# experimental-design/everest

Hardware: AMD Instinct MI355X
Metric: QnehviStrategy.ask() candidates/sec + GP posterior ms, n=512 d=6 m=5 (higher is better)
Workload: dtype f64; 1 GPU; full QnehviStrategy.ask() of BASELINE configs[3] (config 4): DTLZ2(d=6,m=5), n_train=512, S=256 MC samples, 1024 raw Sobol candidates + 20 L-BFGS-B restarts, q=1; value = (raw + optimiser evaluations x batch) / ask wall time, SURVEY.md §8(d); n_train=512, d=6, m=5, mc_samples=256, raw_samples=1024, restarts=20, batch_limit=20, parallelism=1 rank

## Files before the change

### everest_amd/_native.py

```python
from __future__ import annotations

import ctypes
import os
from ctypes import POINTER, c_char_p, c_double, c_int, c_longlong, c_void_p

import torch

_HERE = os.path.dirname(os.path.abspath(__file__))
LIB_PATH = os.environ.get("EVR_LIB_PATH") or os.path.join(_HERE, "_lib", "libeverest_amd.so")

c_double_p = c_void_p
c_int_p = c_void_p


class NativeLibraryError(RuntimeError):
    pass


class EvrQnehviState(ctypes.Structure):
    _fields_ = [
        ("n", c_int), ("nb", c_int), ("S", c_int), ("m", c_int),
        ("c", c_void_p), ("ym", c_void_p), ("ys", c_void_p), ("kxx", c_void_p),
        ("zq", c_void_p), ("obj_a", c_void_p), ("obj_b", c_void_p),
        ("cell_lo", c_void_p), ("cell_hi", c_void_p), ("cell_off", c_void_p), ("max_cells", c_int),
        ("cell_keys", c_void_p), ("cell_pts", c_void_p), ("cell_rank0", c_void_p), ("pts_stride", c_int),
        ("grp_off", c_void_p), ("grp_keys", c_void_p), ("grp_rank", c_void_p), ("grp_box", c_void_p),
        ("sorted_lo", c_void_p), ("max_groups", c_int), ("scan_counters", c_void_p), ("no_h", c_int),
        ("log_hvi", c_int), ("tau_relu", c_double), ("tau_max", c_double),
    ]


class EvrQnehviModel(ctypes.Structure):
    _fields_ = [
        ("n", c_int), ("d", c_int), ("kind", c_int),
        ("Xn", c_void_p), ("lengthscales", c_void_p), ("shift", c_void_p), ("scale", c_void_p), ("M", c_void_p),
    ]


class EvrQnGeneral(ctypes.Structure):
    _fields_ = [
        ("q", c_int), ("m_obj", c_int),
        ("obj_out", c_void_p), ("obj_kind", c_void_p), ("obj_p0", c_void_p), ("obj_p1", c_void_p),
        ("n_con", c_int),
        ("con_out", c_void_p), ("con_sign", c_void_p), ("con_thr", c_void_p), ("con_eta", c_void_p),
        ("zq", c_void_p),
    ]

class EvrNei(ctypes.Structure):
    _fields_ = [
        ("log", c_int), ("tau_relu", c_double), ("tau_max", c_double), ("best", c_void_p), ("best_stride", c_int),
    ]


class EvrSobo(ctypes.Structure):
    _fields_ = [
        ("log", c_int), ("tau_relu", c_double), ("tau_max", c_double), ("best", c_void_p), ("best_stride", c_int),
        ("n_term", c_int),
        ("term_out", c_void_p), ("term_kind", c_void_p), ("term_w", c_void_p), ("term_p0", c_void_p),
        ("term_p1", c_void_p), ("term_p2", c_void_p),
        ("n_con", c_int),
        ("con_out", c_void_p), ("con_sign", c_void_p), ("con_thr", c_void_p), ("con_eta", c_void_p),
    ]


_SIGS = {
    "evr_version": ([], c_int),
    "evr_last_error": ([], c_char_p),
    "evr_device_arch": ([c_int, c_char_p, c_int], c_int),
    "evr_stream_sync": ([c_void_p], c_int),
    "evr_kernel_matrix": ([c_void_p, c_int, c_int, c_int, c_int, c_int] + [c_void_p] * 10, c_int),
    "evr_kernel_cross_grad": ([c_void_p, c_int, c_int, c_int, c_int, c_int] + [c_void_p] * 11, c_int),
    "evr_kernel_cross_grad_workspace_doubles": ([c_int, c_int, c_int], c_longlong),
    "evr_kernel_lengthscale_grad": ([c_void_p, c_int, c_int, c_int, c_int, c_void_p, c_void_p, c_void_p,
                                     c_void_p, c_void_p], c_int),
    "evr_gp_mll_terms": ([c_void_p, c_int, c_int] + [c_void_p] * 5, c_int),
    "evr_gemm_f64": ([c_void_p, c_int, c_int, c_int, c_int, c_int, c_double, c_void_p, c_int, c_longlong,
                      c_void_p, c_int, c_longlong, c_double, c_void_p, c_int, c_longlong, c_int], c_int),
    "evr_cholesky": ([c_void_p, c_int, c_int, c_void_p, c_int, c_longlong, c_void_p, c_int, c_longlong,
                      c_double, c_int, c_void_p, c_void_p], c_int),
    "evr_cholesky_inverse": ([c_void_p, c_int, c_int, c_void_p, c_int, c_longlong, c_void_p, c_int, c_longlong,
                              c_void_p, c_int, c_longlong, c_double, c_int, c_void_p, c_void_p], c_int),
    "evr_trsm_lower":([c_void_p, c_int, c_int, c_int, c_void_p, c_int, c_longlong, c_int, c_void_p, c_int,
                        c_longlong], c_int),
    "evr_tri_inv_lower": ([c_void_p, c_int, c_int, c_void_p, c_int, c_longlong, c_void_p, c_int, c_longlong],
                          c_int),
    "evr_gp_posterior_finalize": ([c_void_p, c_int, c_int, c_int] + [c_void_p] * 8, c_int),
    "evr_gp_posterior_workspace_doubles": ([c_int, c_int, c_int], c_longlong),
    "evr_gp_posterior": ([c_void_p, c_int, c_int, c_int, c_int, c_int] + [c_void_p] * 14, c_int),
    "evr_qnehvi_samples": ([c_void_p, POINTER(EvrQnehviState), c_int, c_void_p, c_void_p, c_void_p, c_void_p],
                           c_int),
    "evr_hvi_workspace_doubles": ([POINTER(EvrQnehviState), c_int, c_int], c_longlong),
    "evr_hvi_forward": ([c_void_p, POINTER(EvrQnehviState), c_int, c_void_p, c_void_p, c_void_p, c_void_p],
                        c_int),
    "evr_mean_over_samples": ([c_void_p, c_int, c_int, c_void_p, c_void_p], c_int),
    "evr_hvi_backward": ([c_void_p, POINTER(EvrQnehviState), c_int, c_void_p, c_void_p, c_void_p, c_void_p],
                         c_int),
    "evr_qnehvi_samples_backward": ([c_void_p, POINTER(EvrQnehviState), c_int, c_void_p, c_void_p, c_void_p,
                                     c_void_p], c_int),
    "evr_pareto_mask": ([c_void_p, c_int, c_int, c_int, c_void_p, c_void_p, c_int, c_void_p, c_void_p], c_int),
    "evr_objective_affine": ([c_void_p, c_int, c_int, c_int] + [c_void_p] * 5, c_int),
    "evr_qei": ([c_void_p, c_int, c_int, c_int, c_void_p, c_double, c_double, c_double, c_double, c_void_p,
                 c_double, c_double, c_double, c_void_p, c_void_p, c_void_p], c_int),
    "evr_scale_batched":([c_void_p, c_int, c_longlong, c_void_p, c_void_p], c_int),
    "evr_add_selection": ([c_void_p, c_int, c_int, c_int, c_void_p, c_void_p, c_void_p], c_int),
    "evr_box_decompose": ([c_int, c_int, c_int, c_void_p, c_longlong, c_longlong, c_longlong, c_void_p,
                           c_void_p, c_int, POINTER(c_void_p)], c_int),
    "evr_box_decompose_approx": ([c_int, c_int, c_int, c_void_p, c_longlong, c_longlong, c_longlong, c_void_p,
                                  c_void_p, c_double, c_int, POINTER(c_void_p)], c_int),
    "evr_cells_total": ([c_void_p], c_longlong),
    "evr_cells_copy": ([c_void_p, c_void_p, c_void_p, c_void_p], c_int),
    "evr_cells_free": ([c_void_p], None),
    "evr_box_device_limits": ([c_int, c_int, c_void_p, c_void_p], c_int),
    "evr_box_device_workspace_bytes": ([c_int, c_int, c_int, c_int], c_longlong),
    "evr_box_decompose_device": ([c_void_p, c_int, c_int, c_int, c_void_p, c_void_p, c_int, c_void_p, c_void_p,
                                  c_void_p], c_int),
    "evr_box_pack_keys_device": ([c_void_p, c_int, c_int, c_int, c_int, c_void_p, c_void_p, c_int, c_void_p,
                                  c_void_p, c_void_p], c_int),
    "evr_box_kd_pipeline": ([c_void_p, c_int, c_int, c_int, c_void_p, c_void_p, c_int] + [c_void_p] * 8
                            + [c_int] + [c_void_p] * 6, c_int),
    "evr_cells_from_keys": ([c_void_p, c_int, c_int, c_int, c_void_p, c_int] + [c_void_p] * 5, c_int),
    "evr_hvi_forward_backward": ([c_void_p, POINTER(EvrQnehviState), c_int] + [c_void_p] * 6, c_int),
    "evr_hvi_restart_fb_applies": ([POINTER(EvrQnehviState), c_int], c_int),
    "evr_hvi_scan_limits": ([c_int, c_int], c_int),
    "evr_hvi_restart_fb": ([c_void_p, POINTER(EvrQnehviState), c_int] + [c_void_p] * 3, c_int),
    "evr_qnehvi_norms_rows": ([POINTER(EvrQnehviState)], c_int),
    "evr_qnehvi_project": ([c_void_p, POINTER(EvrQnehviState), c_int] + [c_void_p] * 5, c_int),
    "evr_qnehvi_project_workspace_doubles": ([POINTER(EvrQnehviState), c_int], c_longlong),
    "evr_qnehvi_samples_norms": ([c_void_p, POINTER(EvrQnehviState), c_int] + [c_void_p] * 5, c_int),
    "evr_qnehvi_project_backward": ([c_void_p, POINTER(EvrQnehviState), c_int] + [c_void_p] * 6, c_int),
    "evr_qnehvi_project_backward_workspace_doubles": ([POINTER(EvrQnehviState), c_int], c_longlong),
    "evr_qnehvi_plan_workspace_bytes": ([POINTER(EvrQnehviState), POINTER(EvrQnehviModel), c_int, c_int],
                                        c_longlong),
    "evr_qnehvi_plan_create": ([c_void_p, POINTER(EvrQnehviState), POINTER(EvrQnehviModel), c_int, c_int, c_void_p,
                               c_void_p, c_void_p, c_void_p, c_int, POINTER(c_void_p)], c_int),
    "evr_qnehvi_plan_run": ([c_void_p, c_void_p], c_int),
    "evr_qnehvi_small_applies": ([POINTER(EvrQnehviState), c_int, c_int], c_int),
    "evr_qnehvi_small_workspace_doubles": ([POINTER(EvrQnehviState), c_int, c_int, c_int], ctypes.c_longlong),
    "evr_qnehvi_small_forward": ([c_void_p, POINTER(EvrQnehviState), POINTER(EvrQnehviModel), c_int, c_void_p,
                                  c_void_p, c_void_p], c_int),
    "evr_qnehvi_small_samples": ([c_void_p, POINTER(EvrQnehviState), c_int, c_void_p, c_void_p, c_void_p, c_void_p,
                                  c_void_p], c_int),
    "evr_qnehvi_small_backward": ([c_void_p, POINTER(EvrQnehviState), POINTER(EvrQnehviModel), c_int, c_void_p,
                                   c_void_p, c_void_p, c_void_p, c_void_p, c_void_p], c_int),
    "evr_mll_plan_create": ([c_void_p, c_int, c_int, c_int, c_int, c_void_p, c_void_p, c_void_p], c_int),
    "evr_mll_plan_eval": ([c_void_p, c_void_p, c_void_p, c_void_p], c_int),
    "evr_mll_plan_destroy": ([c_void_p], None),
    "evr_mll_fit_rounds": ([c_void_p, c_void_p, c_void_p] + [c_void_p] * 7 + [c_int, c_int, c_void_p, c_void_p,
                                                                             c_void_p], c_int),
    "evr_mll_assemble": ([c_int, c_int, c_int] + [c_void_p] * 6, c_int),
    "evr_lbfgsb_advance": ([c_void_p, c_double] + [c_void_p] * 6 + [c_int, c_int], c_int),
    "evr_qnehvi_plan_eval_host": ([c_void_p, c_void_p, c_void_p, c_void_p], c_int),
    "evr_qnehvi_plan_destroy": ([c_void_p], None),
    "evr_lbfgsb_create": ([c_int, c_int, c_void_p, c_void_p, c_double, c_double, c_int, POINTER(c_void_p)], c_int),
    "evr_lbfgsb_start": ([c_void_p, c_void_p, c_void_p], c_int),
    "evr_lbfgsb_step": ([c_void_p, c_double, c_void_p, c_void_p], c_int),
    "evr_lbfgsb_stats": ([c_void_p, c_void_p, c_void_p, c_void_p, c_void_p], None),
    "evr_lbfgsb_destroy": ([c_void_p], None),
    "evr_hit_and_run": ([c_int, c_int, c_void_p, c_void_p, c_int, c_void_p, c_void_p, c_longlong, ctypes.c_ulonglong,
                         c_longlong, c_longlong, c_void_p], c_int),
    "evr_qnehvi_plan_minimize": ([c_void_p, c_void_p, c_void_p, c_void_p, c_void_p, c_int, c_int, c_double,
                                  c_double, c_int, c_int, c_void_p, c_void_p, c_void_p], c_int),
    "evr_qng_workspace_doubles": ([POINTER(EvrQnehviState), POINTER(EvrQnehviState), POINTER(EvrQnGeneral),
                                   POINTER(EvrQnehviModel), c_int, c_int], c_longlong),
    "evr_qng_eval": ([c_void_p, POINTER(EvrQnehviState), POINTER(EvrQnehviState), POINTER(EvrQnGeneral),
                      POINTER(EvrQnehviModel), c_int] + [c_void_p] * 5, c_int),
    "evr_qlog_workspace_doubles": ([POINTER(EvrQnehviState), POINTER(EvrQnehviState), POINTER(EvrQnGeneral),
                                    POINTER(EvrQnehviModel), c_int, c_int], ctypes.c_longlong),
    "evr_qlog_eval": ([c_void_p, POINTER(EvrQnehviState), POINTER(EvrQnehviState), POINTER(EvrQnGeneral),
                       POINTER(EvrQnehviModel), c_int] + [c_void_p] * 5, c_int),
    "evr_nei_scan": ([c_void_p, c_int, c_int, c_int, c_int, c_void_p, c_void_p, c_int, c_double, c_double, c_double,
                      c_double, c_void_p, c_void_p, c_void_p, c_void_p], c_int),
    "evr_qnei_workspace_doubles": ([POINTER(EvrQnehviState), POINTER(EvrQnGeneral), POINTER(EvrQnehviModel), c_int,
                                    c_int], c_longlong),
    "evr_qnei_eval": ([c_void_p, POINTER(EvrQnehviState), POINTER(EvrQnGeneral), POINTER(EvrQnehviModel),
                       POINTER(EvrNei), c_int] + [c_void_p] * 5, c_int),
    "evr_sobo_scan": ([c_void_p, c_int, c_int, c_int, c_int, POINTER(EvrSobo)] + [c_void_p] * 5, c_int),
    "evr_qsobo_workspace_doubles": ([POINTER(EvrQnehviState), POINTER(EvrQnGeneral), POINTER(EvrQnehviModel), c_int,
                                     c_int], c_longlong),
    "evr_qsobo_eval": ([c_void_p, POINTER(EvrQnehviState), POINTER(EvrQnGeneral), POINTER(EvrQnehviModel),
                        POINTER(EvrSobo), c_int] + [c_void_p] * 5, c_int),
    "evr_objective_general": ([c_void_p, c_int, c_int, c_int, POINTER(EvrQnGeneral)] + [c_void_p] * 4, c_int),
    "evr_objective_weights": ([c_void_p, c_int, c_int, POINTER(EvrQnGeneral)] + [c_void_p] * 3, c_int),
    "evr_cells_kd_limits": ([c_int, c_int, c_int, c_void_p], c_int),
    "evr_cells_kd_order_device": ([c_void_p, c_int, c_int, c_int, c_void_p, c_void_p, c_int] + [c_void_p] * 7,
                                  c_int),
    "evr_sobol_scramble": ([c_int, ctypes.c_ulonglong, c_void_p, c_void_p], c_int),
    "evr_sobol_scramble_range": ([c_int, ctypes.c_ulonglong, c_int, c_int, c_void_p, c_void_p], c_int),
    "evr_sobol_stream_words": ([c_int], ctypes.c_longlong),
    "evr_sobol_stream_create": ([ctypes.c_ulonglong, ctypes.c_longlong, c_void_p], c_int),
    "evr_sobol_scramble_stream": ([c_void_p, c_int, c_int, c_int, c_void_p, c_void_p], c_int),
    "evr_sobol_stream_destroy": ([c_void_p], None),
    "evr_sobol_normal": ([c_void_p, c_int, c_int, c_int, c_void_p, c_void_p, c_int, c_int, c_void_p], c_int),
}

EXPORTED_SYMBOLS = tuple(_SIGS)

_lib = None


def load() -> ctypes.CDLL:
    global _lib
    if _lib is not None:
        return _lib
    if not os.path.exists(LIB_PATH):
        raise NativeLibraryError(
            f"everest_amd native library not found at {LIB_PATH}; build it with "
            "`python -c 'import __graft_entry__ as g; g.build()'` (hipcc --offload-arch=gfx950)."
        )
    lib = ctypes.CDLL(LIB_PATH, mode=ctypes.RTLD_GLOBAL)
    for name, (args, res) in _SIGS.items():
        fn = getattr(lib, name)
        fn.argtypes = args
        fn.restype = res
    _lib = lib
    return lib


def check(status: int, what: str = ""):
    if status != 0:
        msg = load().evr_last_error().decode(errors="replace")
        raise RuntimeError(f"everest_amd {what} failed (status {status}): {msg}")


def call(name: str, *args):
    lib = load()
    check(getattr(lib, name)(*args), name)
```

### everest_amd/acquisition.py

```python
from __future__ import annotations

import ctypes
import math
import os
import warnings
from dataclasses import dataclass
from typing import Optional, Sequence

import numpy as np
import torch

from . import _native, ops
from .gp import GPBatch


def sobol_base_samples(S: int, n_points: int, m: int, seed: int, device, scrambled=None) -> torch.Tensor:
    return ops.sobol_normal(S, n_points * m, seed, device, layout=1, m=m, scrambled=scrambled)


_SCRAMBLE_POOL = None


def _prefetch_scramble(dim: int, seed: int, d0: int = 0, nd: Optional[int] = None):
    global _SCRAMBLE_POOL
    nd = dim - d0 if nd is None else nd
    if nd <= 0:
        return None
    key = (int(dim), int(seed), int(d0), int(nd))
    fut = _PREFETCHED.pop(key, None)
    if fut is not None:
        return fut
    if _SCRAMBLE_POOL is None:
        from concurrent.futures import ThreadPoolExecutor

        _SCRAMBLE_POOL = ThreadPoolExecutor(max_workers=3, thread_name_prefix="evr-sobol")
    return _SCRAMBLE_POOL.submit(ops.sobol_scramble, dim, seed, d0, nd)


_PREFETCHED = {}


def prefetch_scramble(dim: int, seed: int, d0: int = 0, nd: Optional[int] = None) -> None:
    nd = dim - d0 if nd is None else nd
    key = (int(dim), int(seed), int(d0), int(nd))
    if nd <= 0 or key in _PREFETCHED:
        return
    while len(_PREFETCHED) >= 8:
        _PREFETCHED.pop(next(iter(_PREFETCHED)))
    _PREFETCHED[key] = _prefetch_scramble(dim, seed, d0, nd)


def _submit(fn, *args):
    global _SCRAMBLE_POOL
    if _SCRAMBLE_POOL is None:
        from concurrent.futures import ThreadPoolExecutor

        _SCRAMBLE_POOL = ThreadPoolExecutor(max_workers=3, thread_name_prefix="evr-sobol")
    return _SCRAMBLE_POOL.submit(fn, *args)


def _prefetch_from_stream(fut_stream, dim: int, d0: int = 0, nd: Optional[int] = None):
    nd = dim - d0 if nd is None else nd
    if nd <= 0:
        return None
    return _submit(lambda: fut_stream.result().scramble(dim, d0, nd))


def _result(fut):
    return None if fut is None else fut.result()


def _host_threads() -> int:
    v = os.environ.get("EVR_HOST_THREADS") or os.environ.get("OMP_NUM_THREADS")
    try:
        return max(1, int(v)) if v else min(16, os.cpu_count() or 1)
    except ValueError:
        return 1


def _single_cell(ref: torch.Tensor, S: int, m: int) -> ops.Cells:
    dev = ref.device
    return ops.Cells(torch.arange(S + 1, dtype=torch.int32, device=dev), np.ones(S, dtype=np.int64), m,
                     lo=ref.unsqueeze(0).repeat(S, 1).contiguous(),
                     hi=torch.full((S, m), math.inf, dtype=torch.float64, device=dev))


def _decompose(O: torch.Tensor, ref: torch.Tensor, box_device=None, kd_scan=None, num_threads=None,
               alpha: float = 0.0):
    m, P, _ = O.shape
    dev = O.device
    approx = alpha > 0.0 and m > 2
    if approx and box_device:
        raise ValueError("the device box decomposition is exact only (alpha = 0)")
    if not approx and (box_device if box_device is not None else
                       ops.box_device_supported(P, m) and ops.hvi_scan_supported(P + m, m)):
        kd_built = False
        try:
            if kd_scan is False or os.environ.get("EVR_BOX_PIPELINE", "1") == "0":
                cells = ops.box_decompose_device(O, ref)
            else:
                cells, kd_built = ops.box_decompose_kd_device(O, ref, want_kd=True)
        except ops.BoxCapacityError as e:
            if box_device:
                raise
            warnings.warn(f"{e}; using the exact host partition", RuntimeWarning)
            cells = None
        if cells is not None:
            path = "device"
            if kd_built:
                path = "device+kd"
            elif kd_scan if kd_scan is not None else ops.kd_supported(cells):
                ops.cells_kd_order(cells)
                path = "device+kd"
            elif kd_scan is None:
                warnings.warn(f"{int(cells.counts.max())} cells in one sample exceed the sparse kd scan's limit; "
                              "using the dense tiled scan (~10x slower)", RuntimeWarning)
            return cells, path
    elif not approx and box_device is None:
        warnings.warn(f"{P} points x {m} objectives exceed the device box decomposition's limits; "
                      "using the host partition", RuntimeWarning)
    mask, _ = ops.pareto_mask(O, ref, dedup=True)
    lo, hi, off = ops.box_decompose(O.cpu().numpy(), ref.cpu().numpy(), mask.cpu().numpy(),
                                    num_threads or _host_threads(), layout="jis", alpha=alpha if approx else 0.0)
    f64 = dict(dtype=torch.float64, device=dev)
    return ops.Cells(torch.as_tensor(off, dtype=torch.int32, device=dev), np.diff(off), m,
                     lo=torch.as_tensor(lo, **f64), hi=torch.as_tensor(hi, **f64)), \
        ("host-approx" if approx else "host")


_BOX_POOL = None
_SIDE_STREAMS = {}


def _decompose_async(O: torch.Tensor, ref: torch.Tensor, *args):
    global _BOX_POOL
    if os.environ.get("EVR_BOX_OVERLAP", "1") == "0" or not O.is_cuda:
        res = _decompose(O, ref, *args)
        return lambda: res
    dev = O.device
    main = torch.cuda.current_stream(dev)
    side = _SIDE_STREAMS.get(dev)
    if side is None:
        side = _SIDE_STREAMS[dev] = torch.cuda.Stream(dev)
    ready = torch.cuda.Event()
    ready.record(main)
    O.record_stream(side)
    ref.record_stream(side)
    if _BOX_POOL is None:
        from concurrent.futures import ThreadPoolExecutor

        _BOX_POOL = ThreadPoolExecutor(max_workers=1, thread_name_prefix="evr-box")

    def job():
        with torch.cuda.device(dev), torch.cuda.stream(side):
            side.wait_event(ready)
            return _decompose(O, ref, *args)

    fut = _BOX_POOL.submit(job)

    def join():
        cells, path = fut.result()
        main.wait_stream(side)
        ts = [cells.off, cells.lo, cells.hi, cells.keys, cells.pts, cells.rank0]
        if cells.kd is not None:
            kd = cells.kd
            ts += [kd.goff, kd.keys, kd.rank, kd.box, kd.sorted_lo]
        for t in ts:
            if isinstance(t, torch.Tensor) and t.is_cuda:
                t.record_stream(main)
        return cells, path

    return join


def _make_spec(m: int, obj_a, obj_b, objective, constraints) -> ops.GeneralSpec:
    if objective is None:
        a = np.asarray(obj_a, dtype=np.float64).reshape(-1)
        b = np.asarray(obj_b, dtype=np.float64).reshape(-1)
        if a.shape[0] != m or b.shape[0] != m:
            raise ValueError(f"obj_a / obj_b need one entry per model output ({m})")
        objective = [(j, ops.OBJ_AFFINE, a[j], b[j]) for j in range(m)]
    return ops.GeneralSpec(m, objective, constraints or ())


def _fast_affine(spec: ops.GeneralSpec, m: int, dev):
    f64 = dict(dtype=torch.float64, device=dev)
    if spec.affine_identity:
        return (torch.tensor([o[2] for o in spec.objectives], **f64),
                torch.tensor([o[3] for o in spec.objectives], **f64))
    return torch.ones(m, **f64), torch.zeros(m, **f64)


@dataclass
class ConstructionStats:
    n_train: int
    n_base: int
    total_cells: int
    max_cells: int
    prune_probs: Optional[np.ndarray] = None


class _BoxHviAcqf:

    @property
    def ref_point(self) -> torch.Tensor:
        return self.ref

    @property
    def constraints(self) -> list:
        return list(self.spec.constraints)

    @property
    def eta(self) -> Optional[torch.Tensor]:
        cs = self.spec.constraints
        if not cs:
            return None
        e = torch.tensor([c[3] for c in cs], dtype=torch.float64)
        return e[0] if len(set(c[3] for c in cs)) == 1 else e

    def _use_log_scan(self, tau_relu: float, tau_max: float):
        if not (tau_relu > 0 and tau_max > 0):
            raise ValueError("tau_relu and tau_max must be positive")
        lo, hi = self.cells.explicit()

        def logify(src):
            st = _native.EvrQnehviState.from_buffer_copy(src)
            st.cell_lo, st.cell_hi = lo.data_ptr(), hi.data_ptr()
            st.log_hvi, st.tau_relu, st.tau_max = 1, float(tau_relu), float(tau_max)
            return st
        self._log_cells = (lo, hi)
        self.state_scan = logify(self.state_scan)
        self.state = logify(self.state)
        if self.spec.affine_identity:
            self.state_model = self.state
        self.tau_relu, self.tau_max = float(tau_relu), float(tau_max)
        self.log_acqf = True
        self._plans = {}

    @property
    def supports_plan(self) -> bool:
        return self.spec.affine_identity and self._pending_rows() is None

    def _init_general(self, spec: ops.GeneralSpec, cells, nk: int, nb_rows: int, no_h: bool = False):
        gp, m = self.gp, self.m
        self.spec = spec
        self._zq_cache = {}
        if spec.affine_identity:
            self.state_model = self.state_scan = self.state
        else:
            ones = torch.ones(max(m, spec.m_obj), dtype=torch.float64, device=self.dev)
            self._dummy = (ones, torch.zeros_like(ones))
            self.state_model = ops.make_state(nk, nb_rows, self.S, m, gp.const, gp.ym, gp.ys, gp.kxx, self.zq,
                                              ones, ones, cells, no_h=no_h)
            self.state_scan = ops.make_state(nk, nb_rows, self.S, spec.m_obj, ones, ones, ones, ones, self.zq,
                                             ones, ones, cells, no_h=no_h)

    def _zq(self, q: int) -> torch.Tensor:
        z = self._zq_cache.get(q)
        if z is None:
            z = self._draw_zq(q).to(dtype=torch.float64, device=self.dev).reshape(self.S, q, self.m).contiguous()
            self._zq_cache[q] = z
        return z

    def set_new_point_samples(self, q: int, z: torch.Tensor):
        self._zq_cache[int(q)] = z.to(dtype=torch.float64, device=self.dev).reshape(self.S, q, self.m).contiguous()

    def _pending_rows(self) -> Optional[torch.Tensor]:
        return None

    def _general(self, X: torch.Tensor, backward: bool, gout: Optional[torch.Tensor] = None):
        b, q, d = X.shape
        Xp = self._pending_rows()
        qq = q
        if Xp is not None:
            X = torch.cat([X, Xp.unsqueeze(0).expand(b, Xp.shape[0], d)], 1)
            qq = X.shape[1]
        if qq > ops.QNG_MAX_Q:
            raise ValueError(f"joint batch of {qq} points (q + pending) exceeds the device limit of {ops.QNG_MAX_Q} "
                             f"(the inclusion-exclusion runs over all 2^q - 1 subsets)")
        g = self.spec.struct(qq, self._zq(qq))
        ev = ops.qlog_eval if getattr(self, "log_acqf", False) else ops.qng_eval
        acq, dX = ev(self.state_model, self.state_scan, g, self.model, X.reshape(b * qq, d).contiguous(),
                     backward, gout)
        if dX is not None:
            dX = dX.view(b, qq, d)[:, :q].contiguous()
        return acq, dX

    def _device_tensors(self):
        out, seen = [], set()

        def walk(v, depth=0):
            if isinstance(v, torch.Tensor):
                if v.device.type == "cuda" and id(v) not in seen:
                    seen.add(id(v))
                    out.append(v)
            elif depth >= 4 or id(v) in seen:
                return
            elif isinstance(v, (list, tuple)):
                for x in v:
                    walk(x, depth + 1)
            elif isinstance(v, dict):
                for x in v.values():
                    walk(x, depth + 1)
            elif type(v).__module__.startswith("everest_amd") and hasattr(v, "__dict__"):
                seen.add(id(v))
                for k, x in vars(v).items():
                    if k not in ("_torch_acqs", "_plans"):
                        walk(x, depth + 1)
        walk(self)
        return out

    def _torch_acq(self, q: int, fast: bool):
        from . import torch_ops

        torch_ops.load()
        cache = self.__dict__.setdefault("_torch_acqs", {})
        acq = cache.get(fast)
        if acq is None:
            def raw(st):
                return torch.frombuffer(bytearray(bytes(st)), dtype=torch.uint8)
            stm = self.state if fast else self.state_model
            sth = self.state if fast else self.state_scan
            acq = torch.classes.everest_amd.QnehviAcq(raw(stm), raw(sth), raw(self.model), bool(fast),
                                                      bool(getattr(self, "log_acqf", False)), self._device_tensors())
            cache[fast] = acq
        done = self.__dict__.setdefault("_torch_general_q", set())
        if not fast and q not in done:
            spec = self.spec
            oo, ok, p0, p1 = spec._arrs
            cons = spec.constraints
            co = torch.tensor([c[0] for c in cons], dtype=torch.int32)
            cs, ct, ce = (torch.tensor([c[k] for c in cons], dtype=torch.float64) for k in (1, 2, 3))
            acq.set_general(int(q), torch.from_numpy(oo), torch.from_numpy(ok), torch.from_numpy(p0),
                            torch.from_numpy(p1), co, cs, ct, ce, self._zq(q))
            done.add(q)
        return acq

    def __call__(self, X: torch.Tensor) -> torch.Tensor:
        from .torch_ops import QnehviFunction

        X3, _ = self._split(X)
        if self._fast(X3):
            return QnehviFunction.apply(X3[:, 0].contiguous(), self._torch_acq(1, True))
        Xp = self._pending_rows()
        if Xp is not None:
            X3 = torch.cat([X3, Xp.unsqueeze(0).expand(X3.shape[0], Xp.shape[0], X3.shape[2])], 1)
        if X3.shape[1] > ops.QNG_MAX_Q:
            raise ValueError(f"joint batch of {X3.shape[1]} points (q + pending) exceeds the device limit of "
                             f"{ops.QNG_MAX_Q} (the inclusion-exclusion runs over all 2^q - 1 subsets)")
        return QnehviFunction.apply(X3.contiguous(), self._torch_acq(X3.shape[1], False))

    def _split(self, X: torch.Tensor):
        X = X.to(device=self.dev, dtype=torch.float64)
        if X.dim() == 2:
            return X.unsqueeze(1), True
        if X.dim() != 3:
            raise ValueError(f"candidates must be b x d or b x q x d, got {tuple(X.shape)}")
        return X, False

    def _fast(self, X3: torch.Tensor) -> bool:
        return X3.shape[1] == 1 and self.supports_plan and self._pending_rows() is None

    def plan(self, b: int, backward: bool) -> ops.QnehviPlan:
        if not self.supports_plan:
            raise NotImplementedError("the native plan covers q = 1 with affine objectives on every output")
        key = (int(b), bool(backward))
        p = self._plans.get(key)
        if p is None:
            if len(self._plans) >= 8:
                self._plans.pop(next(iter(self._plans)))
            p = ops.QnehviPlan(self.state, self.model, int(b), bool(backward), self.dev,
                               graph=os.environ.get("EVR_GRAPH", "1") != "0")
            self._plans[key] = p
        return p

    def forward(self, X: torch.Tensor, return_cache: bool = False):
        if return_cache:
            return self.forward_ops(X, return_cache=True)
        X3, _ = self._split(X)
        if not self._fast(X3):
            return self._general(X3, False)[0]
        p = self.plan(X3.shape[0], False)
        p.X.copy_(X3[:, 0])
        p.run()
        return p.acq.clone()

    def forward_backward(self, X: torch.Tensor, gout: Optional[torch.Tensor] = None):
        X3, flat = self._split(X)
        if not self._fast(X3):
            acq, dX = self._general(X3, True, gout)
            return acq, (dX[:, 0] if flat else dX)
        if gout is not None:
            acq, dX = self.forward_backward_ops(X3[:, 0], gout)
            return acq, (dX if flat else dX.unsqueeze(1))
        p = self.plan(X3.shape[0], True)
        p.X.copy_(X3[:, 0])
        p.run()
        return p.acq.clone(), (p.dX.clone() if flat else p.dX.clone().unsqueeze(1))

    def eval_host(self, x: np.ndarray, backward: bool):
        b = x.shape[0]
        if x.ndim == 2 and self.supports_plan and self._pending_rows() is None:
            out = self.plan(b, backward).run_host(x)
            acq = out[:b].copy()
            return acq, (out[b:].reshape(b, -1).copy() if backward else None)
        Xt = torch.as_tensor(x, dtype=torch.float64, device=self.dev)
        if backward:
            a, g = self.forward_backward(Xt)
            return a.cpu().numpy(), g.cpu().numpy()
        return self.forward(Xt).cpu().numpy(), None

    def _cross(self, X: torch.Tensor) -> torch.Tensor:
        gp = self.gp
        return ops.kernel_matrix(self.Xk, X, gp.ls, gp.kind, shift2=gp.lo, scale2=gp.inv_range)

    def forward_ops(self, X: torch.Tensor, return_cache: bool = False):
        X = X.to(device=self.dev, dtype=torch.float64).contiguous()
        b = X.shape[0]
        Kx = self._cross(X)
        R, P = ops.qnehvi_project(self.state, self.M, Kx, b)
        G, L22, flags = ops.qnehvi_samples_norms(self.state, R, P, b)
        acq = ops.hvi_forward(self.state, G, b, flags)
        if return_cache:
            return acq, (X, R, G, L22, flags)
        return acq

    def forward_backward_ops(self, X: torch.Tensor, gout: Optional[torch.Tensor] = None):
        X = X.to(device=self.dev, dtype=torch.float64).contiguous()
        b = X.shape[0]
        Kx = self._cross(X)
        R, P = ops.qnehvi_project(self.state, self.M, Kx, b)
        G, L22, flags = ops.qnehvi_samples_norms(self.state, R, P, b)
        acq, dG = ops.hvi_forward_backward(self.state, G, b, flags, gout)
        dKx = ops.qnehvi_project_backward(self.state, self.M, R, L22, dG, b)
        gp = self.gp
        dX = ops.kernel_cross_grad(self.Xk, X, gp.ls, dKx, gp.kind, shift2=gp.lo, scale2=gp.inv_range)
        return acq, dX


class QNEHVI(_BoxHviAcqf):

    def __init__(self, gp: GPBatch, X_train_raw: np.ndarray, X_baseline_raw: np.ndarray, ref_point, obj_a, obj_b,
                 S: int = 512, sampler_seed: int = 0, prune_baseline: bool = True, prune_seed: int = 0,
                 prune_samples: int = 2048, max_frac: float = 1.0, z_prune: Optional[torch.Tensor] = None,
                 z_base_full: Optional[torch.Tensor] = None, z_new_full: Optional[torch.Tensor] = None,
                 num_threads: Optional[int] = None, box_device: Optional[bool] = None,
                 kd_scan: Optional[bool] = None, X_pending_raw: Optional[np.ndarray] = None,
                 root: Optional[str] = None, objective=None, constraints=(), alpha: float = 0.0):
        dev = gp.device
        self.gp = gp
        self.dev = dev
        m = gp.B
        n = gp.n
        self.m, self.n, self.S = m, n, int(S)
        f64 = dict(dtype=torch.float64, device=dev)
        spec = _make_spec(m, obj_a, obj_b, objective, constraints)
        self.spec = spec
        self.ref = torch.as_tensor(np.asarray(ref_point, dtype=np.float64), **f64)
        if self.ref.numel() != spec.m_obj:
            raise ValueError(f"reference point has {self.ref.numel()} entries for {spec.m_obj} objectives")
        self.obj_a, self.obj_b = _fast_affine(spec, m, dev)
        self.sampler_seed = int(sampler_seed)
        self._z_new_full = z_new_full
        X_train_raw = np.asarray(X_train_raw, dtype=np.float64)
        X_baseline_raw = np.asarray(X_baseline_raw, dtype=np.float64)
        nbl = X_baseline_raw.shape[0]
        def _distinct_rows(a):
            a = np.ascontiguousarray(a)
            if not np.isfinite(a).all() or np.any((a == 0) & np.signbit(a)):
                return False
            return len(np.unique(a.view(np.dtype((np.void, a.dtype.itemsize * a.shape[1]))))) == a.shape[0]

        all_rows = gp.valid_all_rows() if hasattr(gp, "valid_all_rows") else np.ones(X_train_raw.shape[0], bool)
        if (nbl <= X_train_raw.shape[0] and X_baseline_raw.ndim == 2 and X_baseline_raw.shape[1] > 0
                and np.array_equal(X_baseline_raw, X_train_raw[:nbl]) and _distinct_rows(X_baseline_raw)
                and all_rows[:nbl].all()):
            base_rows = np.arange(nbl, dtype=np.int64)
        else:
            first = {}
            for i, row in enumerate(map(tuple, X_train_raw)):
                if all_rows[i]:
                    first.setdefault(row, i)
            try:
                base_rows = np.array([first[tuple(r)] for r in X_baseline_raw], dtype=np.int64)
            except KeyError as e:
                raise ValueError("qNEHVI: every baseline point must be a training point of the models") from e

        npend = 0 if X_pending_raw is None else int(np.asarray(X_pending_raw).shape[0])
        self.n_pending = npend
        if npend > 0:
            Xp = torch.as_tensor(np.asarray(X_pending_raw, dtype=np.float64).reshape(npend, gp.d), **f64)
            self.Xk = torch.cat([gp.Xn, (Xp - gp.lo) * gp.inv_range], 0).contiguous()
        else:
            self.Xk = gp.Xn
        nk = n + npend
        self.nk = nk

        import time as _time
        tm = {}
        t0 = _time.perf_counter()
        _probe_on = os.environ.get("EVR_CONSTRUCTION_PROBES") == "1"
        _last = [t0]

        def probe(name):
            if _probe_on:
                torch.cuda.synchronize(dev)
                t = _time.perf_counter()
                tm["probe_" + name] = t - _last[0]
                _last[0] = t
        fut_prune = (_prefetch_scramble(len(base_rows) * m, prune_seed)
                     if prune_baseline and z_prune is None else None)
        max_dim = (len(base_rows) + npend + 1) * m
        def _stream_job(after=fut_prune if _host_threads() < 4 else None):
            if after is not None:
                after.result()
            return ops.SobolStream(int(sampler_seed), max_dim)

        fut_stream = (_submit(_stream_job)
                      if max_dim <= ops.SOBOL_MAXDIM and (z_new_full is None or z_base_full is None) else None)
        K = ops.kernel_matrix(self.Xk, self.Xk, gp.ls, gp.kind) if npend else gp.kernel_train(noise=False)
        Kt = K[:, :, :n].contiguous() if npend else K
        mu_t = ops.gemm(Kt, gp.alpha.unsqueeze(-1))[..., 0]
        mu_train = gp.ym[:, None] + gp.ys[:, None] * (gp.const[:, None] + mu_t)
        A = ops.gemm(gp.Linv, K[:, :n].contiguous() if npend else K)
        Sig = ops.gemm(A, A, transA=True, alpha=-1.0, beta=1.0, out=K)
        ops.scale_batched(Sig, (gp.ys ** 2).contiguous())
        probe("joint_posterior")

        probs = None
        if prune_baseline:
            cand = torch.as_tensor(base_rows, device=dev)
            Sig_c = Sig[:, cand][:, :, cand].contiguous()
            mu_c = mu_train[:, cand].contiguous()
            nc = cand.shape[0]
            Lp, _, _ = ops.cholesky(Sig_c, 1e-8, 3)
            probe("prune_chol")
            if z_prune is None:
                Zp = sobol_base_samples(prune_samples, nc, m, prune_seed, dev, _result(fut_prune))
            else:
                Zp = z_prune.to(dev).permute(2, 1, 0).contiguous()
            probe("prune_sobol")
            Yp = ops.gemm(Lp, Zp)
            Op = self._objective(Yp, mu_c)
            _, counts = ops.pareto_mask(Op, self.ref, dedup=False, want_mask=False, want_counts=True)
            probs = counts.cpu().numpy().astype(np.float64) / Zp.shape[2]
            tm["prune"] = _time.perf_counter() - t0
            keep = np.nonzero(probs)[0]
            max_points = math.ceil(max_frac * nc)
            if keep.shape[0] > max_points:
                order = np.argsort(-probs, kind="stable")
                keep = order[:max_points]
            keep = np.unique(keep)
            base_rows = base_rows[keep]
        nb_t = int(base_rows.shape[0])
        if npend:
            base_rows = np.concatenate([base_rows, n + np.arange(npend, dtype=np.int64)])
        nb = int(base_rows.shape[0])
        self.nb = nb
        self.base_rows = base_rows
        idx = torch.as_tensor(base_rows, device=dev)
        S_ = self.S
        if fut_stream is not None:
            fut_q = _prefetch_from_stream(fut_stream, (nb + 1) * m, nb * m, m) if z_new_full is None else None
            fut_b = (_prefetch_from_stream(fut_stream, nb_t * m)
                     if nb > 0 and nb_t > 0 and z_base_full is None else None)
        else:
            fut_q = _prefetch_scramble((nb + 1) * m, sampler_seed, nb * m, m) if z_new_full is None else None
            fut_b = _prefetch_scramble(nb_t * m, sampler_seed) if nb > 0 and z_base_full is None else None

        if nb > 0:
            Sig_b = Sig[:, idx][:, :, idx].contiguous()
            self.L_base, self.base_jitter, _ = ops.cholesky(Sig_b, 1e-8, 3)
            mu_b = mu_train[:, idx].contiguous()
            probe("baseline_chol")
        if z_new_full is None:
            self.zq = ops.sobol_normal(S_, (nb + 1) * m, sampler_seed, dev, d0=nb * m, nd=m,
                                       scrambled=_result(fut_q))
        else:
            self.zq = z_new_full[:, nb, :].to(**f64).contiguous()
        if nb > 0:
            if z_base_full is None:
                Zb = sobol_base_samples(S_, nb_t, m, sampler_seed, dev, _result(fut_b))
                if npend:
                    Zp_ = ops.sobol_normal(S_, nb * m, sampler_seed, dev, d0=nb_t * m, nd=npend * m, layout=1, m=m)
                    Zb = torch.cat([Zb, Zp_], 1).contiguous()
            else:
                Zb = z_base_full.to(dev).permute(2, 1, 0).contiguous()
            self._Zb = Zb
            probe("baseline_sobol")
            Yb = ops.gemm(self.L_base, Zb)
            Ob = self._objective(Yb, mu_b)
            tm["baseline"] = _time.perf_counter() - t0 - tm.get("prune", 0.0)
            t1 = _time.perf_counter()
            join_box = _decompose_async(Ob, self.ref, box_device, kd_scan, num_threads, alpha) \
                if not _probe_on else (lambda r: (lambda: r))(_decompose(Ob, self.ref, box_device, kd_scan,
                                                                         num_threads, alpha))
        else:
            cells0 = _single_cell(self.ref, S_, spec.m_obj)
            join_box = lambda: (cells0, "none")
        probe("box")

        root = root or os.environ.get("EVR_ROOT", "split")
        if root not in ("fused", "split"):
            raise ValueError(f"root must be 'fused' or 'split', got {root!r}")
        fused = root == "fused" and nb > 0
        self.root = "fused" if fused else "split"
        nb_rows = 0 if fused else nb
        Rr = nk + nb_rows + S_ + 1
        self.Rr = Rr
        M = torch.zeros(m, Rr, nk, **f64) if npend else torch.empty(m, Rr, n, **f64)
        M[:, :n, :n].copy_(gp.Linv)
        if nb > 0:
            A_b = A[:, :, idx].contiguous()
            E = ops.gemm(A_b, gp.Linv, transA=True, alpha=-1.0)
            if npend:
                E = torch.cat([E, torch.zeros(m, nb, npend, **f64)], 2).contiguous()
            ops.add_selection(E, idx.to(torch.int32), None)
            ops.scale_batched(E, (gp.ys ** 2).contiguous())
            ops.trsm(self.L_base, E)
            ops.gemm_into(M[:, nk + nb_rows:nk + nb_rows + S_], Zb, E, transA=True)
            if fused:
                if npend:
                    Lp = torch.zeros(m, nk, nk, **f64)
                    Lp[:, :n, :n].copy_(gp.L)
                    Lpi = torch.zeros(m, nk, nk, **f64)
                    Lpi[:, :n, :n].copy_(gp.Linv)
                    Lp[:, n:, n:].copy_(torch.eye(npend, **f64))
                    Lpi[:, n:, n:].copy_(torch.eye(npend, **f64))
                else:
                    Lp, Lpi = gp.L, gp.Linv
                ops.scale_batched(E, (1.0 / gp.ys).contiguous())
                V = ops.gemm(E, Lp)
                Iv = ops.gemm(V, V, transA=True)
                Iv.diagonal(dim1=-2, dim2=-1)[:, :n] += 1.0
                probe("root_gemms")
                Lv, _, _ = ops.cholesky(Iv, 1e-8, 3)
                probe("root_chol")
                ops.gemm_into(M[:, :nk], Lv, Lpi, transA=True)
            else:
                M[:, nk:nk + nb].copy_(E)
        else:
            M[:, nk:nk + S_].zero_()
        cells, self.box_path = join_box()
        if nb > 0:
            tm["box_decomposition"] = _time.perf_counter() - t1
        self.cells = cells
        counts_c = cells.counts
        self.stats = ConstructionStats(n_train=n, n_base=nb, total_cells=int(np.sum(counts_c)),
                                       max_cells=int(counts_c.max()) if len(counts_c) else 0, prune_probs=probs)
        M[:, Rr - 1, :n].copy_(gp.alpha)
        self.M = M
        self.state = ops.make_state(nk, nb_rows, S_, m, gp.const, gp.ym, gp.ys, gp.kxx, self.zq, self.obj_a,
                                    self.obj_b, cells)
        self._keep = (self.zq, self.obj_a, self.obj_b)
        self._init_general(spec, cells, nk, nb_rows)
        if not spec.affine_identity:
            self.state = self.state_scan
        self._lo_c = gp.lo.to(torch.float64).contiguous()
        self._scale_c = gp.inv_range.to(torch.float64).contiguous()
        self.model = _native.EvrQnehviModel(n=nk, d=gp.d, kind=gp.kind, Xn=self.Xk.data_ptr(), lengthscales=gp.ls.data_ptr(),
                                            shift=self._lo_c.data_ptr(), scale=self._scale_c.data_ptr(),
                                            M=self.M.data_ptr())
        probe("operator")
        self._plans = {}
        torch.cuda.synchronize(dev)
        tm["total"] = _time.perf_counter() - t0
        self.timings = tm


    def z_base_host(self) -> Optional[torch.Tensor]:
        zb = getattr(self, "_Zb", None)
        return None if zb is None else zb.permute(2, 1, 0).cpu().contiguous()

    def _objective(self, Y: torch.Tensor, mu: torch.Tensor) -> torch.Tensor:
        if self.spec.affine_identity:
            return ops.objective_affine(Y, mu, self.obj_a, self.obj_b)
        return ops.objective_general(Y, mu, self.spec, self.ref)

    def _draw_zq(self, q: int) -> torch.Tensor:
        nb, m = self.nb, self.m
        if self._z_new_full is not None:
            if self._z_new_full.shape[1] < nb + q:
                raise ValueError(f"z_new_full has {self._z_new_full.shape[1]} rows, need {nb + q}")
            return self._z_new_full[:, nb:nb + q, :]
        return ops.sobol_normal(self.S, (nb + q) * m, self.sampler_seed, self.dev, d0=nb * m, nd=q * m)


class QEHVI(_BoxHviAcqf):

    def __init__(self, gp: GPBatch, Y_part: np.ndarray, ref_point, obj_a, obj_b, S: int = 512,
                 sampler_seed: int = 0, z: Optional[torch.Tensor] = None, box_device: Optional[bool] = None,
                 kd_scan: Optional[bool] = None, num_threads: Optional[int] = None, objective=None,
                 constraints=(), X_pending_raw: Optional[np.ndarray] = None, alpha: float = 0.0):
        dev = gp.device
        self.gp, self.dev = gp, dev
        m, n = gp.B, gp.n
        self.m, self.n, self.S, self.nb, self.nk = m, n, int(S), 0, n
        f64 = dict(dtype=torch.float64, device=dev)
        spec = _make_spec(m, obj_a, obj_b, objective, constraints)
        self.spec = spec
        mo = spec.m_obj
        self.ref = torch.as_tensor(np.asarray(ref_point, dtype=np.float64), **f64)
        if self.ref.numel() != mo:
            raise ValueError(f"reference point has {self.ref.numel()} entries for {mo} objectives")
        self.obj_a, self.obj_b = _fast_affine(spec, m, dev)
        self.sampler_seed = int(sampler_seed)
        Y_part = np.asarray(Y_part, dtype=np.float64).reshape(-1, mo)
        self.Y_part = Y_part
        self.Xk = gp.Xn
        S_ = self.S
        if Y_part.shape[0] > 0:
            O = torch.as_tensor(np.ascontiguousarray(Y_part.T), **f64)[:, :, None].expand(mo, Y_part.shape[0], S_)
            cells, self.box_path = _decompose(O.contiguous(), self.ref, box_device, kd_scan, num_threads, alpha)
        else:
            cells, self.box_path = _single_cell(self.ref, S_, mo), "none"
        self.cells = cells
        cnt = cells.counts
        self.stats = ConstructionStats(n_train=n, n_base=0, total_cells=int(np.sum(cnt)),
                                       max_cells=int(cnt.max()) if len(cnt) else 0)
        self._z1 = z
        if z is None:
            self.zq = ops.sobol_normal(S_, m, sampler_seed, dev)
        else:
            self.zq = z.reshape(S_, m).to(**f64).contiguous()
        self.X_pending = None
        if X_pending_raw is not None and np.asarray(X_pending_raw).shape[0] > 0:
            self.X_pending = torch.as_tensor(np.asarray(X_pending_raw, dtype=np.float64).reshape(-1, gp.d), **f64)
        self.Rr = n + 1
        M = torch.empty(m, n + 1, n, **f64)
        M[:, :n].copy_(gp.Linv)
        M[:, n].copy_(gp.alpha)
        self.M = M
        self.state = ops.make_state(n, 0, S_, m, gp.const, gp.ym, gp.ys, gp.kxx, self.zq, self.obj_a, self.obj_b,
                                    cells, no_h=True)
        self._lo_c = gp.lo.to(torch.float64).contiguous()
        self._scale_c = gp.inv_range.to(torch.float64).contiguous()
        self.model = _native.EvrQnehviModel(n=n, d=gp.d, kind=gp.kind, Xn=self.Xk.data_ptr(),
                                            lengthscales=gp.ls.data_ptr(), shift=self._lo_c.data_ptr(),
                                            scale=self._scale_c.data_ptr(), M=self.M.data_ptr())
        self._plans = {}
        self._init_general(spec, cells, n, 0, no_h=True)
        if not spec.affine_identity:
            self.state = self.state_scan
        torch.cuda.synchronize(dev)

    def _pending_rows(self) -> Optional[torch.Tensor]:
        return self.X_pending

    def _draw_zq(self, q: int) -> torch.Tensor:
        if q == 1 and self._z1 is not None:
            return self.zq
        return ops.sobol_normal(self.S, q * self.m, self.sampler_seed, self.dev)


TAU_RELU = 1e-6
TAU_MAX_MO = 1e-3


class QLogNEHVI(QNEHVI):

    def __init__(self, *args, tau_relu: float = TAU_RELU, tau_max: float = TAU_MAX_MO, **kw):
        super().__init__(*args, **kw)
        self._use_log_scan(tau_relu, tau_max)


class QLogEHVI(QEHVI):

    def __init__(self, *args, tau_relu: float = TAU_RELU, tau_max: float = TAU_MAX_MO, **kw):
        super().__init__(*args, **kw)
        self._use_log_scan(tau_relu, tau_max)


class QEIJoint(QEHVI):

    def __init__(self, gp: GPBatch, X_train_raw: np.ndarray, obj_a: float, obj_b: float, S: int = 512,
                 seed: int = 0, X_pending_raw: Optional[np.ndarray] = None):
        if gp.B != 1:
            raise ValueError("QEIJoint takes a single-output model")
        Xt = torch.as_tensor(np.asarray(X_train_raw, dtype=np.float64), device=gp.device)
        mean, _ = gp.posterior(Xt)
        best_f = float((float(obj_a) * mean[0] + float(obj_b)).max().item())
        super().__init__(gp, np.array([[best_f]]), [best_f - 1.0], [float(obj_a)], [float(obj_b)], S=S,
                         sampler_seed=seed, box_device=False, X_pending_raw=X_pending_raw)
        self.best_f = best_f
        self.a, self.b = float(obj_a), float(obj_b)


TAU_MAX_SO = 1e-2


class _NeiAcqf(_BoxHviAcqf):

    @property
    def supports_plan(self) -> bool:
        return False

    def _finish(self, obj_a: float, obj_b: float, no_h: bool, log: bool, tau_relu: float, tau_max: float,
                X_pending_raw):
        gp = self.gp
        f64 = dict(dtype=torch.float64, device=self.dev)
        if log and not (tau_relu > 0 and tau_max > 0):
            raise ValueError("tau_relu and tau_max must be positive")
        self.m, self.n, self.nk = 1, gp.n, gp.n
        self.a, self.b = float(obj_a), float(obj_b)
        self.log_acqf = bool(log)
        self.tau_relu, self.tau_max = float(tau_relu), float(tau_max)
        self.spec = ops.GeneralSpec(1, [(0, ops.OBJ_AFFINE, self.a, self.b)])
        self.X_pending = None
        if X_pending_raw is not None and np.asarray(X_pending_raw).shape[0] > 0:
            self.X_pending = torch.as_tensor(np.asarray(X_pending_raw, dtype=np.float64).reshape(-1, gp.d), **f64)
        self.n_pending = 0 if self.X_pending is None else int(self.X_pending.shape[0])
        self.Xk = gp.Xn
        self.Rr = gp.n + self.nb + (0 if no_h else self.S) + 1
        self.state = ops.model_state(gp.n, self.nb, self.S, gp.const, gp.ym, gp.ys, gp.kxx, no_h=no_h)
        self._lo_c = gp.lo.to(torch.float64).contiguous()
        self._scale_c = gp.inv_range.to(torch.float64).contiguous()
        self.model = _native.EvrQnehviModel(n=gp.n, d=gp.d, kind=gp.kind, Xn=self.Xk.data_ptr(),
                                            lengthscales=gp.ls.data_ptr(), shift=self._lo_c.data_ptr(),
                                            scale=self._scale_c.data_ptr(), M=self.M.data_ptr())
        self.best = self.best.to(**f64).reshape(-1).contiguous()
        self.nei = ops.nei_struct(log, tau_relu, tau_max, self.best)
        self._zq_cache = {}
        self._plans = {}
        torch.cuda.synchronize(self.dev)

    def _pending_rows(self) -> Optional[torch.Tensor]:
        return self.X_pending

    def _joint(self, X: torch.Tensor) -> torch.Tensor:
        Xp = self.X_pending
        if Xp is not None:
            X = torch.cat([X, Xp.unsqueeze(0).expand(X.shape[0], Xp.shape[0], X.shape[2])], 1)
        if X.shape[1] > ops.QNG_MAX_Q:
            raise ValueError(f"joint batch of {X.shape[1]} points (q + pending) exceeds the device limit of "
                             f"{ops.QNG_MAX_Q}")
        return X

    def _general(self, X: torch.Tensor, backward: bool, gout: Optional[torch.Tensor] = None):
        b, q, d = X.shape
        X = self._joint(X)
        qq = X.shape[1]
        g = self.spec.struct(qq, self._zq(qq))
        acq, dX = ops.qnei_eval(self.state, g, self.model, self.nei, X.reshape(b * qq, d).contiguous(), backward,
                                gout)
        if dX is not None:
            dX = dX.view(b, qq, d)[:, :q].contiguous()
        return acq, dX

    def _torch_acq(self, q: int, fast: bool = False):
        from . import torch_ops

        torch_ops.load()
        acq = self.__dict__.get("_torch_nei")
        if acq is None:
            def raw(st):
                return torch.frombuffer(bytearray(bytes(st)), dtype=torch.uint8)
            acq = torch.classes.everest_amd.QneiAcq(raw(self.state), raw(self.model), self.log_acqf, self.tau_relu,
                                                    self.tau_max, self.best, self.a, self.b, self._device_tensors())
            self._torch_nei = acq
        done = self.__dict__.setdefault("_torch_nei_q", set())
        if q not in done:
            acq.set_samples(int(q), self._zq(q))
            done.add(q)
        return acq

    def __call__(self, X: torch.Tensor) -> torch.Tensor:
        from .torch_ops import QneiFunction

        X3 = self._joint(self._split(X)[0]).contiguous()
        return QneiFunction.apply(X3, self._torch_acq(X3.shape[1]))


class QNEI(_NeiAcqf):

    _LOG = False

    def __init__(self, gp: GPBatch, X_train_raw: np.ndarray, X_baseline_raw: np.ndarray, obj_a: float, obj_b: float,
                 S: int = 512, sampler_seed: int = 0, prune_baseline: bool = True, prune_seed: int = 0,
                 prune_samples: int = 2048, z_prune: Optional[torch.Tensor] = None,
                 X_pending_raw: Optional[np.ndarray] = None, tau_relu: float = TAU_RELU,
                 tau_max: float = TAU_MAX_SO):
        if gp.B != 1:
            raise ValueError(f"{type(self).__name__} takes a single-output model")
        dev = gp.device
        self.gp, self.dev, self.S = gp, dev, int(S)
        self.sampler_seed = int(sampler_seed)
        n, S_ = gp.n, self.S
        f64 = dict(dtype=torch.float64, device=dev)
        a_t = torch.tensor([float(obj_a)], **f64)
        b_t = torch.tensor([float(obj_b)], **f64)
        first = {}
        for i, row in enumerate(map(tuple, np.asarray(X_train_raw, dtype=np.float64))):
            first.setdefault(row, i)
        try:
            base_rows = np.array([first[tuple(r)] for r in np.asarray(X_baseline_raw, dtype=np.float64)],
                                 dtype=np.int64)
        except KeyError as e:
            raise ValueError("qNEI: every baseline point must be a training point of the model") from e
        if base_rows.shape[0] == 0:
            raise ValueError("qNEI needs a non-empty baseline")
        K = gp.kernel_train(noise=False)
        mu_t = ops.gemm(K, gp.alpha.unsqueeze(-1))[..., 0]
        mu_train = gp.ym[:, None] + gp.ys[:, None] * (gp.const[:, None] + mu_t)
        A = ops.gemm(gp.Linv, K)
        Sig = ops.gemm(A, A, transA=True, alpha=-1.0, beta=1.0, out=K)
        ys2 = (gp.ys ** 2).contiguous()
        ops.scale_batched(Sig, ys2)
        self.prune_counts = None
        if prune_baseline:
            cand = torch.as_tensor(base_rows, device=dev)
            nc = int(cand.shape[0])
            Lp, _, _ = ops.cholesky(Sig[:, cand][:, :, cand].contiguous(), 1e-8, 3)
            if z_prune is None:
                Zp = sobol_base_samples(prune_samples, nc, 1, prune_seed, dev)
            else:
                Zp = z_prune.to(**f64).reshape(-1, nc, 1).permute(2, 1, 0).contiguous()
            Op = ops.objective_affine(ops.gemm(Lp, Zp), mu_train[:, cand].contiguous(), a_t, b_t)
            _, counts = ops.pareto_mask(Op, torch.full((1,), -math.inf, **f64), dedup=False, want_mask=False,
                                        want_counts=True)
            self.prune_counts = counts.cpu().numpy()
            base_rows = base_rows[np.nonzero(self.prune_counts)[0]]
        nb = int(base_rows.shape[0])
        self.nb, self.base_rows = nb, base_rows
        idx = torch.as_tensor(base_rows, device=dev)
        self.L_base, self.base_jitter, _ = ops.cholesky(Sig[:, idx][:, :, idx].contiguous(), 1e-8, 3)
        Zb = sobol_base_samples(S_, nb, 1, sampler_seed, dev)
        self._Zb = Zb
        Ob = ops.objective_affine(ops.gemm(self.L_base, Zb), mu_train[:, idx].contiguous(), a_t, b_t)
        self.best = Ob[0].amax(0)
        Rr = n + nb + S_ + 1
        M = torch.empty(1, Rr, n, **f64)
        M[:, :n].copy_(gp.Linv)
        E = ops.gemm(A[:, :, idx].contiguous(), gp.Linv, transA=True, alpha=-1.0)
        ops.add_selection(E, idx.to(torch.int32), None)
        ops.scale_batched(E, ys2)
        ops.trsm(self.L_base, E)
        M[:, n:n + nb].copy_(E)
        ops.gemm_into(M[:, n + nb:n + nb + S_], Zb, E, transA=True)
        M[:, Rr - 1].copy_(gp.alpha)
        self.M = M
        self._finish(obj_a, obj_b, False, self._LOG, tau_relu, tau_max, X_pending_raw)

    def z_base_host(self) -> torch.Tensor:
        return self._Zb.permute(2, 1, 0).cpu().contiguous()

    def _draw_zq(self, q: int) -> torch.Tensor:
        return ops.sobol_normal(self.S, self.nb + q, self.sampler_seed, self.dev, d0=self.nb, nd=q)


class QLogNEI(QNEI):

    _LOG = True


class QLogEI(_NeiAcqf):

    def __init__(self, gp: GPBatch, X_train_raw: np.ndarray, obj_a: float, obj_b: float, S: int = 512,
                 seed: int = 0, X_pending_raw: Optional[np.ndarray] = None, tau_relu: float = TAU_RELU,
                 tau_max: float = TAU_MAX_SO, log: bool = True):
        if gp.B != 1:
            raise ValueError("QLogEI takes a single-output model")
        self.gp, self.dev, self.S, self.nb = gp, gp.device, int(S), 0
        self.sampler_seed = int(seed)
        Xt = torch.as_tensor(np.asarray(X_train_raw, dtype=np.float64), device=self.dev)
        mean, _ = gp.posterior(Xt)
        self.best_f = float((float(obj_a) * mean[0] + float(obj_b)).max().item())
        self.best = torch.tensor([self.best_f], dtype=torch.float64, device=self.dev)
        self.M = gp.M
        self._finish(obj_a, obj_b, True, log, tau_relu, tau_max, X_pending_raw)

    def z_base_host(self) -> None:
# ... 239 lines not shown
```

### everest_amd/csrc/box_device.hip

```cpp
#include <algorithm>
#include <cmath>
#include <cstdlib>

#include "common.hpp"
#include "../../include/everest_amd.h"

namespace evr {

constexpr int BD_THREADS = 1024;
constexpr unsigned long long BD_DEAD = ~0ull;
constexpr int BD_LDS_BYTES = 160 * 1024 - 2048;
constexpr int BD_STG = 256;

struct BdLayout {
  long long cap;
  int n, m;
  size_t off_lub, off_buf, off_aidx, off_pts, off_inv0, off_nf, bytes;
};

static BdLayout bd_layout(int S, int n, int m, int cap) {
  BdLayout L;
  L.cap = cap;
  L.n = n;
  L.m = m;
// ... 116 lines not shown
      r += (w > v) || (w == v && k < i);
    }
    inv0[r] = i;
    rank[i] = r;
  }
  __syncthreads();

  int Kend = 1, holes = 0;
  if (tid == 0) {
    unsigned long long k0 = 0;
    k0 = K::set(k0, 0, rank[nf]);
    for (int j = 1; j < M; ++j) k0 = K::set(k0, j, nf + j);
    lub[0] = k0;
  }
  __syncthreads();
  for (int p = 0; p < nf; ++p) {
    double z[M];
#pragma unroll
    for (int j = 0; j < M; ++j) z[j] = pt[p * M + j];
    if (tid == 0) {
      sh_nA = 0;
      sh_nNew = 0;
    }
    __syncthreads();
    for (int u = tid; u < Kend; u += BD_THREADS) {
      const unsigned long long key = lub[u];
      if (key == BD_DEAD) continue;
      bool dom = pt[inv0[K::field(key, 0)] * M] > z[0];
#pragma unroll
      for (int j = 1; j < M; ++j) dom &= pt[K::field(key, j) * M + j] > z[j];
      if (dom) {
        const int k = atomicAdd(&sh_nA, 1);
        if (LS && k < BD_STG) astg[k] = u;
        else aidx[k] = u;
      }
    }
    __syncthreads();
    const int nA = sh_nA;
    for (int t = tid; t < nA * M; t += BD_THREADS) {
      const int a = t / M, j = t - a * M;
      const unsigned long long key = lub[(LS && a < BD_STG) ? astg[a] : aidx[a]];
      double zmax = -INFINITY;
#pragma unroll
      for (int k = 0; k < M; ++k) {
        if (k == j) continue;
        const int pk = (k == 0) ? inv0[K::field(key, 0)] : K::field(key, k);
        zmax = fmax(zmax, pt[pk * M + j]);
      }
      if (z[j] >= zmax) {
        const int slot = atomicAdd(&sh_nNew, 1);
        if (slot < cap) {
          const unsigned long long nk = K::set(key, j, j == 0 ? rank[p] : p);
          if (LS && slot < BD_STG) stg[slot] = nk;
          else buf[slot] = nk;
        }
      }
    }
    __syncthreads();
    const int nNew = sh_nNew;
    if (Kend + (nNew > nA ? nNew - nA : 0) > cap || nNew > cap) {
      if (tid == 0) sh_err = 1;
      break;
    }
    const int top = nNew > nA ? nNew : nA;
    for (int i = tid; i < top; i += BD_THREADS) {
      const bool st = LS && i < BD_STG;
      if (i < nNew) {
        const int dst = (i < nA) ? (st ? astg[i] : aidx[i]) : Kend + (i - nA);
        lub[dst] = st ? stg[i] : buf[i];
      } else {
        lub[st ? astg[i] : aidx[i]] = BD_DEAD;
      }
    }
    if (nNew > nA) Kend += nNew - nA;
    else holes += nA - nNew;
    __syncthreads();
    if (holes > 256 && holes * 4 > Kend) {
      if (tid == 0) sh_cnt = 0;
      __syncthreads();
      for (int u = tid; u < Kend; u += BD_THREADS) {
        const unsigned long long key = lub[u];
        if (key != BD_DEAD) buf[atomicAdd(&sh_cnt, 1)] = key;
      }
      __syncthreads();
      const int cnt = sh_cnt;
      for (int u = tid; u < cnt; u += BD_THREADS) lub[u] = buf[u];
      Kend = cnt;
      holes = 0;
      __syncthreads();
    }
  }
  __syncthreads();
  if (sh_err) {
    if (tid == 0) {
      status[s] = 1;
      counts[s] = 0;
      if (hmap) {
        hmap[s] = 0;
        hmap[S + s] = 1;
      }
    }
    return;
  }

  if (tid == 0) sh_cnt = 0;
  __syncthreads();
  for (int u = tid; u < Kend; u += BD_THREADS) {
    const unsigned long long key = lub[u];
    if (key == BD_DEAD) continue;
    int P[M];
    P[0] = inv0[K::field(key, 0)];
#pragma unroll
    for (int j = 1; j < M; ++j) P[j] = K::field(key, j);
    bool ok = true;
#pragma unroll
    for (int j = 1; j < M; ++j) {
      double lo = -INFINITY;
#pragma unroll
      for (int k = 0; k < j; ++k) lo = fmax(lo, pt[P[k] * M + j]);
      ok &= pt[P[j] * M + j] > lo;
    }
    if (ok) buf[atomicAdd(&sh_cnt, 1)] = key;
  }
  __syncthreads();
  const int C = sh_cnt;
  int P2 = 1;
  while (P2 < C) P2 <<= 1;
  if (P2 <= sortcap) {
    for (int i = tid; i < P2; i += BD_THREADS) sbuf[i] = (i < C) ? buf[i] : BD_DEAD;
    __syncthreads();
    wg_bitonic<unsigned long long, BD_THREADS>(sbuf, P2);
    for (int i = tid; i < C; i += BD_THREADS) buf[i] = sbuf[i];
  } else {
    for (int i = C + tid; i < P2; i += BD_THREADS) buf[i] = BD_DEAD;
    __syncthreads();
    bd_bitonic(buf, P2);
  }
  for (int e = tid; e < (nf + M) * M; e += BD_THREADS) gpts[e] = pt[e];
  for (int r = tid; r <= nf; r += BD_THREADS) ginv0[r] = inv0[r];
  if (tid == 0) {
    counts[s] = C;
    status[s] = 0;
    ((int*)(ws + Lo.off_nf))[s] = nf;
    if (hmap) {
      hmap[s] = C;
      hmap[S + s] = 0;
    }
  }
}

template <int M>
__global__ __launch_bounds__(256) void cells_from_keys_kernel(int stride, const int* __restrict__ off,
                                                              const unsigned long long* __restrict__ keys,
                                                              const double* __restrict__ pts,
                                                              const int* __restrict__ rank0, double* __restrict__ lo,
                                                              double* __restrict__ hi) {
  using K = CellKey<M>;
  const int s = blockIdx.y;
  const int i = blockIdx.x * 256 + threadIdx.x;
  const int c0 = off[s], C = off[s + 1] - c0;
  if (i >= C) return;
  double l[M], h[M];
  K::decode(keys[c0 + i], pts + (size_t)s * stride * M, rank0 + (size_t)s * stride, l, h);
  const size_t o = (size_t)(c0 + i) * M;
#pragma unroll
  for (int j = 0; j < M; ++j) {
    lo[o + j] = l[j];
    hi[o + j] = h[j];
  }
}

template <int M>
__global__ __launch_bounds__(256) void bd_pack_keys_kernel(int S, int n, int cap, const unsigned char* __restrict__ ws,
                                                           BdLayout Lo, const int* __restrict__ off,
                                                           unsigned long long* __restrict__ keys,
                                                           double* __restrict__ pts, int* __restrict__ rank0) {
  const int s = blockIdx.y;
  const int i = blockIdx.x * 256 + threadIdx.x;
  const int c0 = off[s], C = off[s + 1] - c0;
  if (i < C) keys[c0 + i] = ((const unsigned long long*)(ws + Lo.off_buf))[(size_t)s * cap + i];
  if (blockIdx.x == 0) {
    const size_t np = (size_t)(n + M);
    const double* gp = (const double*)(ws + Lo.off_pts) + s * np * M;
    const int* gi = (const int*)(ws + Lo.off_inv0) + s * np;
    const size_t nv = (size_t)((const int*)(ws + Lo.off_nf))[s] + M;
    for (size_t e = threadIdx.x; e < np * M; e += 256) pts[s * np * M + e] = e < nv * M ? gp[e] : INFINITY;
    for (size_t e = threadIdx.x; e < np; e += 256) rank0[s * np + e] = e + M <= nv ? gi[e] : 0;
  }
}

}

using namespace evr;

#define EVR_BD_SWITCH(m, MACRO)                                                       \
  switch (m) {                                                                        \
    case 1: MACRO(1); break;                                                          \
    case 2: MACRO(2); break;                                                          \
    case 3: MACRO(3); break;                                                          \
    case 4: MACRO(4); break;                                                          \
    case 5: MACRO(5); break;                                                          \
    case 6: MACRO(6); break;                                                          \
    case 7: MACRO(7); break;                                                          \
    case 8: MACRO(8); break;                                                          \
    default: EVR_CHECK(false, "box decomposition: m=%d not supported (1..8)", m);     \
  }

extern "C" {

int evr_box_device_limits(int n, int m, int* max_points_out, long long* lds_bytes_out) {
  EVR_CHECK(m >= 1 && m <= 8 && n >= 0, "evr_box_device_limits: bad arguments");
  const long long idx_limit = (1ll << bd_field_bits(m)) - 2 - m;
  const size_t fixed = bd_lds_fixed(n, m);
  if (max_points_out) *max_points_out = (int)std::min<long long>(idx_limit, 1 << 20);
  if (lds_bytes_out) *lds_bytes_out = (long long)fixed;
  return (n <= idx_limit && fixed + 16 + 8 * 64 <= (size_t)BD_LDS_BYTES) ? 0 : 3;
}

long long evr_box_device_workspace_bytes(int S, int n, int m, int cap) {
  if (S < 1 || n < 0 || m < 1 || cap < 1) return 0;
  return (long long)bd_layout(S, n, m, cap).bytes;
}

static int box_decompose_launch(void* stream, int S, int n, int m, const double* obj, const double* ref, int cap,
                                void* work, int* counts, int* status, int* hmap);

int evr_box_decompose_device(void* stream, int S, int n, int m, const double* obj, const double* ref, int cap,
                             void* work, int* counts, int* status) {
  return box_decompose_launch(stream, S, n, m, obj, ref, cap, work, counts, status, nullptr);
}

static int box_decompose_launch(void* stream, int S, int n, int m, const double* obj, const double* ref, int cap,
                                void* work, int* counts, int* status, int* hmap) {
  EVR_CHECK(S >= 1 && n >= 1 && m >= 1 && m <= 8 && obj && ref && work && counts && status,
            "evr_box_decompose_device: bad arguments");
  EVR_CHECK(cap >= 2 && (cap & (cap - 1)) == 0, "evr_box_decompose_device: cap must be a power of two");
  EVR_CHECK(evr_box_device_limits(n, m, nullptr, nullptr) == 0,
            "evr_box_decompose_device: n=%d points x m=%d exceed the device limits", n, m);
  const BdLayout Lo = bd_layout(S, n, m, cap);
  const size_t fixed = bd_lds_fixed(n, m) + 16;
  auto sort_cap = [&](size_t fx) {
    int c = 1;
    while ((size_t)(c * 2) * 8 + fx <= (size_t)BD_LDS_BYTES && c * 2 <= cap) c *= 2;
    return c;
  };
  const size_t fixed_ls = fixed + (size_t)BD_STG * (8 + 4);
  const char* ev = std::getenv("EVR_BD_LDS");
  const bool ls = sort_cap(fixed_ls) >= cap && !(ev && ev[0] == '0');
  const int sortcap = ls ? cap : sort_cap(fixed);
  const size_t lds = (ls ? fixed_ls : fixed) + (size_t)sortcap * 8;
  hipStream_t s = (hipStream_t)stream;
#define L2(MM, LS_)                                                                                          \
  do {                                                                                                       \
    EVR_HIP(hipFuncSetAttribute((const void*)bd_build_kernel<MM, LS_>,                                      \
                                hipFuncAttributeMaxDynamicSharedMemorySize, (int)lds));                      \
    bd_build_kernel<MM, LS_><<<S, BD_THREADS, lds, s>>>(S, n, obj, ref, cap, sortcap, (unsigned char*)work, \
                                                        Lo, counts, status, hmap);                           \
  } while (0)
#define L(MM)            \
  if (ls) L2(MM, true);  \
  else L2(MM, false)
  EVR_BD_SWITCH(m, L);
#undef L
#undef L2
  EVR_LAUNCH_CHECK();
  return 0;
}

int evr_cells_from_keys(void* stream, int S, int m, int stride, const int* off, int max_cells,
                        const unsigned long long* keys, const double* pts, const int* rank0, double* lo,
                        double* hi) {
  EVR_CHECK(S >= 1 && m >= 1 && m <= 8 && stride > m && off && keys && pts && rank0 && lo && hi,
            "evr_cells_from_keys: bad arguments");
  if (max_cells <= 0) return 0;
  dim3 grid(cdiv(max_cells, 256), S);
  hipStream_t s = (hipStream_t)stream;
#define L(MM) cells_from_keys_kernel<MM><<<grid, 256, 0, s>>>(stride, off, keys, pts, rank0, lo, hi)
  EVR_BD_SWITCH(m, L);
#undef L
  EVR_LAUNCH_CHECK();
  return 0;
}

int evr_box_pack_keys_device(void* stream, int S, int n, int m, int cap, const void* work, const int* off,
                             int max_cells, unsigned long long* keys, double* pts, int* rank0) {
  EVR_CHECK(S >= 1 && n >= 1 && m >= 1 && m <= 8 && work && off && keys && pts && rank0,
            "evr_box_pack_keys_device: bad arguments");
  const BdLayout Lo = bd_layout(S, n, m, cap);
  dim3 grid(std::max(1, cdiv(max_cells, 256)), S);
  hipStream_t s = (hipStream_t)stream;
#define L(MM) \
  bd_pack_keys_kernel<MM><<<grid, 256, 0, s>>>(S, n, cap, (const unsigned char*)work, Lo, off, keys, pts, rank0)
  EVR_BD_SWITCH(m, L);
#undef L
  EVR_LAUNCH_CHECK();
  return 0;
}


int evr_box_kd_pipeline(void* stream, int S, int n, int m, const double* obj, const double* ref, int cap,
                        void* work, int* counts_dev, int* status_dev, int* off_dev, int* goff_dev,
                        unsigned long long* keys, double* pts, int* rank0, int want_kd, unsigned long long* okeys,
                        unsigned short* ork, unsigned short* ogb, double* osv, int* counts_host, int* info) {
  EVR_CHECK(S >= 1 && counts_dev && status_dev && off_dev && goff_dev && keys && pts && rank0 && counts_host &&
                info && (!want_kd || (okeys && ork && ogb && osv)),
            "evr_box_kd_pipeline: bad arguments");
  hipStream_t s = (hipStream_t)stream;
  thread_local int* stage = nullptr;
  thread_local int* stage_d = nullptr;
  thread_local size_t stage_n = 0;
  thread_local int stage_dev = -1;
  thread_local hipEvent_t copied = nullptr;
  if (copied) EVR_HIP(hipEventSynchronize(copied));
  int dev = 0;
  EVR_HIP(hipGetDevice(&dev));
  const size_t need = (size_t)4 * S + 2;
  if (stage_n < need || stage_dev != dev) {
    if (copied) {
      (void)hipEventDestroy(copied);
      copied = nullptr;
    }
    if (stage) (void)hipHostFree(stage);
    stage = stage_d = nullptr;
    stage_n = 0;
    stage_dev = -1;
    EVR_HIP(hipHostMalloc((void**)&stage, sizeof(int) * need, hipHostMallocMapped | hipHostMallocCoherent));
    EVR_HIP(hipHostGetDevicePointer((void**)&stage_d, stage, 0));
    stage_n = need;
    stage_dev = dev;
  }
  if (!copied) EVR_HIP(hipEventCreateWithFlags(&copied, hipEventDisableTiming));
  int* hc = stage;
  int* hs = stage + S;
  int* hoff = stage + 2 * S;
  int* hgoff = hoff + S + 1;
  if (int rc = box_decompose_launch(stream, S, n, m, obj, ref, cap, work, counts_dev, status_dev, stage_d)) return rc;
  EVR_HIP(hipStreamSynchronize(s));
  info[0] = info[1] = info[2] = 0;
  int maxc = 0;
  for (int i = 0; i < S; ++i) {
    counts_host[i] = hc[i];
    if (hs[i]) info[0] = 1;
    maxc = std::max(maxc, hc[i]);
  }
  info[2] = maxc;
  if (info[0]) return 0;
  long long c = 0, g = 0;
  for (int i = 0; i < S; ++i) {
    hoff[i] = (int)c;
    hgoff[i] = (int)g;
    c += hc[i];
    g += (hc[i] + 15) / 16;
  }
  hoff[S] = (int)c;
  hgoff[S] = (int)g;
  EVR_CHECK(c <= (long long)S * cap && c < 0x7FFFFFFFLL, "evr_box_kd_pipeline: %lld cells exceed the capacity", c);
  const int* moff = stage_d + 2 * S;
  const int* mgoff = moff + S + 1;
  if (int rc = evr_box_pack_keys_device(stream, S, n, m, cap, work, moff, maxc, keys, pts, rank0)) return rc;
  const int stride = n + m;
  if (want_kd && evr_cells_kd_limits(stride, m, maxc, nullptr) == 0) {
    if (int rc = evr_cells_kd_order_device(stream, S, m, stride, moff, mgoff, maxc, keys, pts, rank0, okeys, ork,
                                           ogb, osv))
      return rc;
    info[1] = 1;
  }
  EVR_HIP(hipMemcpyAsync(off_dev, hoff, sizeof(int) * (S + 1), hipMemcpyHostToDevice, s));
  EVR_HIP(hipMemcpyAsync(goff_dev, hgoff, sizeof(int) * (S + 1), hipMemcpyHostToDevice, s));
  EVR_HIP(hipEventRecord(copied, s));
  return 0;
}

}
```

### everest_amd/csrc/common.hpp

```cpp
#pragma once
#include <hip/hip_runtime.h>

#include <cmath>
#include <cstdarg>
#include <cstdio>
#include <cstring>
#include <string>

namespace evr {

void set_error(const char* fmt, ...);
const char* last_error();

#define EVR_HIP(call)                                                             \
  do {                                                                            \
    hipError_t e_ = (call);                                                       \
    if (e_ != hipSuccess) {                                                       \
      ::evr::set_error("%s:%d %s -> %s", __FILE__, __LINE__, #call,               \
                       hipGetErrorString(e_));                                    \
      return 1;                                                                   \
    }                                                                             \
  } while (0)

#define EVR_CHECK(cond, ...)                                                      \
  do {                                                                            \
    if (!(cond)) {                                                                \
      ::evr::set_error(__VA_ARGS__);                                              \
      return 2;                                                                   \
    }                                                                             \
  } while (0)

#define EVR_LAUNCH_CHECK()                                                        \
  do {                                                                            \
    hipError_t e_ = hipGetLastError();                                            \
    if (e_ != hipSuccess) {                                                       \
      ::evr::set_error("%s:%d kernel launch -> %s", __FILE__, __LINE__,           \
                       hipGetErrorString(e_));                                    \
      return 1;                                                                   \
    }                                                                             \
  } while (0)

inline int cdiv(long long a, long long b) { return (int)((a + b - 1) / b); }

__device__ __forceinline__ int xcd_swizzle(int orig, int nwg) {
  const int xcd = orig & 7, q = nwg >> 3, r = nwg & 7;
  return (xcd < r ? xcd * (q + 1) : r * (q + 1) + (xcd - r) * q) + (orig >> 3);
}

__device__ __constant__ static const double kExp2J64[64] = {
    1.0, 1.0108892860517005, 1.0218971486541166, 1.0330248790212284,
    1.0442737824274138, 1.0556451783605572, 1.0671404006768237, 1.0787607977571199,
    1.0905077326652577, 1.102382583307841, 1.1143867425958924, 1.1265216186082418,
    1.1387886347566916, 1.1511892299529827, 1.1637248587775775, 1.1763969916502812,
    1.189207115002721, 1.202156731452703, 1.215247359980469, 1.22848053610687,
    1.241857812073484, 1.255380757024691, 1.2690509571917332, 1.2828700160787783,
    1.2968395546510096, 1.3109612115247644, 1.3252366431597413, 1.339667524053303,
    1.3542555469368927, 1.3690024229745905, 1.383909881963832, 1.3989796725383112,
    1.4142135623730951, 1.42961333839197, 1.4451808069770467, 1.460917794180647,
    1.4768261459394993, 1.4929077282912648, 1.5091644275934228, 1.5255981507445384,
    1.5422108254079407, 1.559004400237837, 1.5759808451078865, 1.593142151342267,
    1.6104903319492543, 1.6280274218573478, 1.645755478153965, 1.6636765803267364,
    1.681792830507429, 1.7001063537185235, 1.718619298122478, 1.7373338352737062,
    1.7562521603732995, 1.7753764925265212, 1.7947090750031072, 1.8142521755003989,
    1.8340080864093424, 1.8539791250833855, 1.8741676341103, 1.8945759815869656,
    1.9152065613971474, 1.9360617934922943, 1.9571441241754002, 1.978456026387951,
};

__device__ __forceinline__ double exp_k_t(double x, const double* __restrict__ T) {
  x = x < -760.0 ? -760.0 : x;
  const double kd = __builtin_rint(x * 92.33248261689366);
  const int k = (int)kd;
  double r = fma(kd, -0.010830424696249145, x);
  r = fma(kd, -3.623510646634843e-19, r);
  double q = fma(r, 1.0 / 720.0, 1.0 / 120.0);
  q = fma(q, r, 1.0 / 24.0);
  q = fma(q, r, 1.0 / 6.0);
  q = fma(q, r, 0.5);
  const double p = fma(q, r * r, r);
  const double t = T[k & 63];
  return __builtin_ldexp(fma(t, p, t), k >> 6);
}
__device__ __forceinline__ void kexp_stage(double* T, int tid, int nthreads) {
  for (int i = tid; i < 64; i += nthreads) T[i] = kExp2J64[i];
}

__device__ __forceinline__ double exp_k(double x) {
  x = x < -760.0 ? -760.0 : x;
  const double kd = __builtin_rint(x * 92.33248261689366);
  const int k = (int)kd;
  double r = fma(kd, -0.010830424696249145, x);
  r = fma(kd, -3.623510646634843e-19, r);
  double q = fma(r, 1.0 / 720.0, 1.0 / 120.0);
  q = fma(q, r, 1.0 / 24.0);
  q = fma(q, r, 1.0 / 6.0);
  q = fma(q, r, 0.5);
  const double p = fma(q, r * r, r);
  const double t = kExp2J64[k & 63];
  return __builtin_ldexp(fma(t, p, t), k >> 6);
}

template <class State>
inline int qn_nh(const State* st) { return st->no_h ? 0 : st->S; }
template <class State>
inline int qn_rows(const State* st) { return st->n + st->nb + qn_nh(st) + 1; }

enum KernelKind { RBF = 0, MATERN05 = 1, MATERN15 = 2, MATERN25 = 3 };
constexpr int KIND_MIXED = 16, KIND_MAX_MIXED = 13;
__host__ __device__ __forceinline__ int kind_of(int code, int j) {
  return code < KIND_MIXED ? code : (code >> (5 + 2 * j)) & 3;
}
inline bool kind_code_ok(int code, int B) {
  if (code >= 0 && code <= 3) return true;
  if (!(code & KIND_MIXED) || (code & 15) || B < 1 || B > KIND_MAX_MIXED) return false;
  return (code >> (5 + 2 * B)) == 0;
}

__device__ __forceinline__ double kernel_value(int kind, double d2) {
  if (kind == RBF) return exp_k(-0.5 * d2);
  const double d = sqrt(fmax(d2, 1e-30));
  if (kind == MATERN05) return exp_k(-d);
  if (kind == MATERN15) {
    const double s = 1.7320508075688772 * d;
    return (1.0 + s) * exp_k(-s);
  }
  const double s = 2.23606797749979 * d;
  return (1.0 + s + (5.0 / 3.0) * d2) * exp_k(-s);
}
__device__ __forceinline__ double sqrt_pos(double x) {
#pragma clang fp contract(off)
  const double y = __builtin_amdgcn_rsq(x);
  double g = x * y, h = 0.5 * y;
  const double r = fma(-h, g, 0.5);
  g = fma(g, r, g);
  h = fma(h, r, h);
  return fma(fma(-g, g, x), h, g);
}
__device__ __forceinline__ double kernel_value_r(int kind, double d2, const double* __restrict__ T) {
#pragma clang fp contract(off)
  if (kind == RBF) return exp_k_t(-0.5 * d2, T);
  const double d = sqrt_pos(fmax(d2, 1e-30));
  if (kind == MATERN05) return exp_k_t(-d, T);
  if (kind == MATERN15) {
    const double s = 1.7320508075688772 * d;
    return (1.0 + s) * exp_k_t(-s, T);
  }
  const double s = 2.23606797749979 * d;
  return fma(5.0 / 3.0, d2, 1.0 + s) * exp_k_t(-s, T);
}
__device__ __forceinline__ double kernel_value_t(int kind, double d2, const double* __restrict__ T) {
  if (kind == RBF) return exp_k_t(-0.5 * d2, T);
  const double d = sqrt(fmax(d2, 1e-30));
  if (kind == MATERN05) return exp_k_t(-d, T);
  if (kind == MATERN15) {
    const double s = 1.7320508075688772 * d;
    return (1.0 + s) * exp_k_t(-s, T);
  }
  const double s = 2.23606797749979 * d;
  return (1.0 + s + (5.0 / 3.0) * d2) * exp_k_t(-s, T);
}
__device__ __forceinline__ double kernel_dscale_t(int kind, double d2, const double* __restrict__ T) {
  if (kind == RBF) return -exp_k_t(-0.5 * d2, T);
  if (d2 < 1e-30) return 0.0;
  const double d = sqrt(d2);
  if (kind == MATERN05) return -exp_k_t(-d, T) / d;
  if (kind == MATERN15) return -3.0 * exp_k_t(-1.7320508075688772 * d, T);
  const double s = 2.23606797749979 * d;
  return -(5.0 / 3.0) * (1.0 + s) * exp_k_t(-s, T);
}

__device__ __forceinline__ double kernel_dscale(int kind, double d2) {
  if (kind == RBF) return -exp_k(-0.5 * d2);
  if (d2 < 1e-30) return 0.0;
  const double d = sqrt(d2);
  if (kind == MATERN05) return -exp_k(-d) / d;
  if (kind == MATERN15) return -3.0 * exp_k(-1.7320508075688772 * d);
  const double s = 2.23606797749979 * d;
  return -(5.0 / 3.0) * (1.0 + s) * exp_k(-s);
}

__host__ __device__ constexpr int bd_field_bits(int m) { return m <= 4 ? 16 : (m == 5 ? 12 : 64 / m); }

template <int M>
struct CellKey {
  static constexpr int FB = bd_field_bits(M);
  static constexpr unsigned long long FMASK = (1ull << FB) - 1;
  __device__ static int field(unsigned long long k, int j) { return (int)((k >> (FB * (M - 1 - j))) & FMASK); }
  __device__ static unsigned long long set(unsigned long long k, int j, int v) {
    const int sh = FB * (M - 1 - j);
    return (k & ~(FMASK << sh)) | ((unsigned long long)v << sh);
  }
  __device__ static void decode(unsigned long long key, const double* pt, const int* rank0, double* lo,
                                double* hi) {
    int P[M];
    P[0] = rank0[field(key, 0)];
#pragma unroll
    for (int j = 1; j < M; ++j) P[j] = field(key, j);
#pragma unroll
    for (int j = 0; j < M; ++j) {
      double bl = -INFINITY;
#pragma unroll
      for (int k = 0; k < j; ++k) bl = fmax(bl, pt[P[k] * M + j]);
      lo[j] = -pt[P[j] * M + j];
      hi[j] = -bl;
    }
  }
  __device__ static void decode_direct(unsigned long long key, const double* pt, double* lo, double* hi) {
    int P[M];
#pragma unroll
    for (int j = 0; j < M; ++j) P[j] = field(key, j);
#pragma unroll
    for (int j = 0; j < M; ++j) {
      double bl = -INFINITY;
#pragma unroll
      for (int k = 0; k < j; ++k) bl = fmax(bl, pt[P[k] * M + j]);
      lo[j] = -pt[P[j] * M + j];
      hi[j] = -bl;
    }
  }
};

constexpr double HL_UMAX = 1e10;

__device__ __forceinline__ double log_fatplus(double z, double tr, double* dpsi) {
  const double x = z / tr;
  double sp, dsp;
  if (x > 20.0) {
    sp = x;
    dsp = 1.0;
  } else if (x < -60.0) {
    sp = 0.0;
    dsp = 0.0;
  } else {
    const double e = exp(x);
    sp = log1p(e);
    dsp = e / (1.0 + e);
  }
  const double c = 1.0 / (1.0 + x * x);
  const double F = sp + 0.1 * c;
  if (dpsi) *dpsi = (dsp - 0.2 * x * c * c) / (tr * F);
  return log(tr * F);
}

__device__ __forceinline__ double fatmin2(double a, double b, double t, double* da) {
  if (b == -INFINITY) {
    if (da) *da = 0.0;
    return -INFINITY;
  }
  const double x = fabs(a - b) / t;
  const double p = 2.0 / (2.0 + x * (2.0 + x));
  const double dq = p * p * (1.0 + x) / (1.0 + p);
  if (da) *da = (a < b) ? 1.0 - dq : dq;
  return fmin(a, b) - t * log(1.0 + p);
}

struct FastLogTabs {
  double2 li[65];
  double et[64];
  __device__ void fill(int tid, int nthreads) {
    for (int i = tid; i < 65; i += nthreads) {
      li[i] = make_double2(log1p(i / 64.0), 1.0 / (1.0 + i / 64.0));
      if (i < 64) et[i] = exp2(i / 64.0);
    }
  }
};

__device__ __forceinline__ double rcp_nr(double d) {
  double r = __builtin_amdgcn_rcp(d);
  double e = fma(-d, r, 1.0);
  r = fma(r, e, r);
  e = fma(-d, r, 1.0);
  return fma(r, e, r);
}

__device__ __forceinline__ double log1p_tab(double p, const FastLogTabs& T) {
  const int i = min(64, (int)(p * 64.0));
  const double2 L = T.li[i];
  const double r = (p - i * (1.0 / 64.0)) * L.y;
  double q = -1.0 / 8.0;
  q = fma(q, r, 1.0 / 7.0);
  q = fma(q, r, -1.0 / 6.0);
  q = fma(q, r, 1.0 / 5.0);
  q = fma(q, r, -1.0 / 4.0);
  q = fma(q, r, 1.0 / 3.0);
  q = fma(q, r, -1.0 / 2.0);
  q = fma(q, r, 1.0);
  return fma(q, r, L.x);
}

__device__ __forceinline__ double log_tab(double w, const FastLogTabs& T) {
  if (!(w > 0.0)) return -INFINITY;
  int e;
  const double m = 2.0 * frexp(w, &e);
  constexpr double LN2_HI = 6.93147180369123816490e-01, LN2_LO = 1.90821492927058770002e-10;
  const double e1 = (double)(e - 1);
  return fma(e1, LN2_HI, fma(e1, LN2_LO, log1p_tab(m - 1.0, T)));
}

__device__ __forceinline__ double exp_tab_neg(double x, const FastLogTabs& T) {
  if (x < -745.2) return 0.0;
  constexpr double K64 = 92.33248261689365951;
  constexpr double C_HI = 1.08304246962070465088e-02, C_LO = 4.20986316660698181e-14;
  const double kd = rint(x * K64);
  const int k = (int)kd;
  const double r = fma(-kd, C_LO, fma(-kd, C_HI, x));
  double q = 1.0 / 720.0;
  q = fma(q, r, 1.0 / 120.0);
  q = fma(q, r, 1.0 / 24.0);
  q = fma(q, r, 1.0 / 6.0);
  q = fma(q, r, 0.5);
  q = fma(q, r, 1.0);
  const double t = T.et[k & 63];
  return ldexp(fma(t * r, q, t), k >> 6);
}

__device__ __forceinline__ double fatmin_fast(double a, double b, double t, double it, double* da,
                                              const FastLogTabs& T) {
  if (b == -INFINITY) {
    *da = 0.0;
    return -INFINITY;
  }
  const double x = fabs(a - b) * it;
  const double q = fma(x, 2.0 + x, 2.0);
  const double qq = q * (q + 2.0);
  const bool big = isinf(qq);
  const double w = big ? 0.0 : rcp_nr(qq);
  const double p = big ? 0.0 : 2.0 * (q + 2.0) * w;
  const double dq = big ? 0.0 : 4.0 * (1.0 + x) * w;
  *da = (a < b) ? 1.0 - dq : dq;
  return fmin(a, b) - t * log1p_tab(p, T);
}

template <int M, bool BWD>
struct LseState {
  double m, s0, g[BWD ? M : 1];
  __device__ void init() {
    m = -INFINITY;
    s0 = 0.0;
#pragma unroll
    for (int j = 0; j < (BWD ? M : 1); ++j) g[j] = 0.0;
  }
  __device__ void add(double a, const double* da) {
    if (a == -INFINITY) return;
    const double e = exp(-fabs(a - m));
    if (a > m) {
      s0 = fma(s0, e, 1.0);
// ... 132 lines not shown
```

### everest_amd/ops.py

```python
from __future__ import annotations

import ctypes
import os
import warnings
from typing import Optional, Tuple

import numpy as np
import torch

from . import _native
from ._native import EvrQnehviState, EvrQnGeneral, call

KERNELS = {"rbf": 0, "matern05": 1, "matern15": 2, "matern25": 3}
KIND_BY_NU = {0.5: 1, 1.5: 2, 2.5: 3}


class NotPSDError(RuntimeError):
    """Raised when the jitter ladder of psd_safe_cholesky is exhausted ([upstream]
    linear_operator NotPSDError, caught by fit_gpytorch_mll's retries)."""


QNG_MAX_Q = 12

def _stream() -> int:
# ... 618 lines not shown
        call("evr_qnehvi_plan_eval_host", _stream(), self._h, xh.ctypes.data, out.ctypes.data)
        return out

    def minimize(self, x0: np.ndarray, lb: np.ndarray, ub: np.ndarray, maxiter: int, maxfun: int = 15000,
                 maxcor: int = 10, ftol: float = 2.220446049250313e-09, gtol: float = 1e-5, maxls: int = 20):
        if not self.backward:
            raise ValueError("minimize needs a backward plan")
        n = self.b * self.d
        f64 = lambda a: np.ascontiguousarray(np.asarray(a, dtype=np.float64).reshape(n))
        x0, lb, ub = f64(x0), f64(lb), f64(ub)
        x = np.empty(n)
        acq = np.empty(self.b)
        info = np.zeros(4, dtype=np.int32)
        rc = self._lib.evr_qnehvi_plan_minimize(_stream(), self._h, x0.ctypes.data, lb.ctypes.data, ub.ctypes.data,
                                                int(maxiter), int(maxfun), ftol / float(np.finfo(float).eps),
                                                float(gtol), int(maxcor), int(maxls), x.ctypes.data,
                                                acq.ctypes.data, info.ctypes.data)
        if rc == 7:
            raise NotPSDError(self._lib.evr_last_error().decode(errors="replace"))
        _native.check(rc, "evr_qnehvi_plan_minimize")
        return x, acq, info.tolist()

    def __del__(self):
        h = getattr(self, "_h", None)
        if h is not None and h.value:
            self._lib.evr_qnehvi_plan_destroy(h)
            self._h = None


def _hvi_work(st: EvrQnehviState, b: int, backward: bool, device) -> torch.Tensor:
    n = _native.load().evr_hvi_workspace_doubles(ctypes.byref(st), b, int(backward))
    return torch.empty(max(1, n), dtype=torch.float64, device=device)


def hvi_forward(st: EvrQnehviState, G: torch.Tensor, b: int, flags: Optional[torch.Tensor] = None) -> torch.Tensor:
    acq = torch.empty(b, dtype=torch.float64, device=G.device)
    work = _hvi_work(st, b, False, G.device)
    call("evr_hvi_forward", _stream(), ctypes.byref(st), b, G.data_ptr(), _p(flags), work.data_ptr(),
         acq.data_ptr())
    return acq


def mean_over_samples(partial: torch.Tensor):
    S, b = partial.shape
    acq = torch.empty(b, dtype=torch.float64, device=partial.device)
    call("evr_mean_over_samples", _stream(), S, b, partial.data_ptr(), acq.data_ptr())
    return acq


def hvi_backward(st: EvrQnehviState, G: torch.Tensor, gout: Optional[torch.Tensor], b: int):
    dG = torch.empty_like(G)
    if gout is not None:
        gout = _dev(gout, "gout")
    work = _hvi_work(st, b, True, G.device)
    call("evr_hvi_backward", _stream(), ctypes.byref(st), b, G.data_ptr(), _p(gout), work.data_ptr(),
         dG.data_ptr())
    return dG


def hvi_forward_backward(st: EvrQnehviState, G: torch.Tensor, b: int, flags: Optional[torch.Tensor] = None,
                         gout: Optional[torch.Tensor] = None):
    acq = torch.empty(b, dtype=torch.float64, device=G.device)
    dG = torch.empty_like(G)
    if gout is not None:
        gout = _dev(gout, "gout")
    work = _hvi_work(st, b, True, G.device)
    call("evr_hvi_forward_backward", _stream(), ctypes.byref(st), b, G.data_ptr(), _p(flags), _p(gout),
         work.data_ptr(), acq.data_ptr(), dG.data_ptr())
    return acq, dG


def hvi_restart_fb_applies(st: EvrQnehviState, b: int) -> bool:
    return bool(_native.load().evr_hvi_restart_fb_applies(ctypes.byref(st), int(b)))


def hvi_restart_fb(st: EvrQnehviState, G: torch.Tensor, b: int):
    S = int(st.S)
    sval = torch.empty(S, b, dtype=torch.float64, device=G.device)
    dG = torch.empty_like(G)
    call("evr_hvi_restart_fb", _stream(), ctypes.byref(st), b, G.data_ptr(), sval.data_ptr(), dG.data_ptr())
    return sval, dG


def qnehvi_samples_backward(st: EvrQnehviState, R, L22, dG, b: int):
    gR = torch.empty_like(R)
    call("evr_qnehvi_samples_backward", _stream(), ctypes.byref(st), b, R.data_ptr(), L22.data_ptr(), dG.data_ptr(),
         gR.data_ptr())
    return gR


def pareto_mask(O: torch.Tensor, ref: torch.Tensor, dedup: bool, want_mask=True, want_counts=False):
    O, ref = _dev(O, "O"), _dev(ref, "ref")
    m, n, S = O.shape
    mask = torch.empty(S, n, dtype=torch.uint8, device=O.device) if want_mask else None
    counts = torch.zeros(n, dtype=torch.int32, device=O.device) if want_counts else None
    call("evr_pareto_mask", _stream(), S, n, m, O.data_ptr(), ref.data_ptr(), int(dedup), _p(mask), _p(counts))
    return mask, counts


def objective_affine(Y: torch.Tensor, mu: Optional[torch.Tensor], a: torch.Tensor, b: torch.Tensor):
    Y = _dev(Y, "Y")
    m, n, S = Y.shape
    O = torch.empty_like(Y)
    mu = None if mu is None else _dev(mu, "mu")
    call("evr_objective_affine", _stream(), m, n, S, Y.data_ptr(), _p(mu), _dev(a, "a").data_ptr(),
         _dev(b, "b").data_ptr(), O.data_ptr())
    return O


def qei(R: torch.Tensor, c: float, ym: float, ys: float, kxx: float, z: torch.Tensor, a: float, b: float,
        best_f: float, with_grad: bool):
    R, z = _dev(R, "R"), _dev(z, "z")
    n1, nb = R.shape
    acq = torch.empty(nb, dtype=torch.float64, device=R.device)
    gR = torch.empty_like(R) if with_grad else None
    flags = torch.empty(nb, dtype=torch.int32, device=R.device)
    call("evr_qei", _stream(), n1 - 1, nb, z.numel(), R.data_ptr(), float(c), float(ym), float(ys), float(kxx),
         z.data_ptr(), float(a), float(b), float(best_f), acq.data_ptr(), _p(gR), flags.data_ptr())
    return acq, gR, flags


def scale_batched(X: torch.Tensor, alpha: torch.Tensor) -> torch.Tensor:
    if not X.is_contiguous():
        raise ValueError("scale_batched: X must be contiguous")
    B = X.shape[0]
    call("evr_scale_batched", _stream(), B, X.numel() // B, _dev(alpha, "alpha").data_ptr(), X.data_ptr())
    return X


def add_selection(E: torch.Tensor, idx: torch.Tensor, val: Optional[torch.Tensor]) -> torch.Tensor:
    B, nb, n = E.shape
    idx = _dev(idx, "idx", torch.int32)
    call("evr_add_selection", _stream(), B, nb, n, idx.data_ptr(), _p(None if val is None else _dev(val, "val")),
         E.data_ptr())
    return E


def box_device_supported(n: int, m: int) -> bool:
    return _native.load().evr_box_device_limits(int(n), int(m), None, None) == 0


def hvi_scan_supported(stride: int, m: int) -> bool:
    return _native.load().evr_hvi_scan_limits(int(stride), int(m)) == 0


class Cells:

    def __init__(self, off, counts, m, lo=None, hi=None, keys=None, pts=None, rank0=None, stride=0):
        self.off, self.counts, self.m = off, np.asarray(counts, dtype=np.int64), int(m)
        self.lo, self.hi, self.keys, self.pts, self.rank0, self.stride = lo, hi, keys, pts, rank0, int(stride)
        self.kd: Optional[KdGroups] = None

    @property
    def S(self) -> int:
        return int(self.counts.shape[0])

    @property
    def total(self) -> int:
        return int(self.counts.sum())

    @property
    def max_cells(self) -> int:
        return int(self.counts.max()) if self.S else 0

    def explicit(self) -> Tuple[torch.Tensor, torch.Tensor]:
        if self.keys is None:
            return self.lo, self.hi
        lo = torch.empty(self.total, self.m, dtype=torch.float64, device=self.off.device)
        hi = torch.empty_like(lo)
        call("evr_cells_from_keys", _stream(), self.S, self.m, self.stride, self.off.data_ptr(), self.max_cells,
             self.keys.data_ptr(), self.pts.data_ptr(), self.rank0.data_ptr(), lo.data_ptr(), hi.data_ptr())
        return lo, hi


class KdGroups:

    def __init__(self, goff, keys, rank, box, sorted_lo, max_groups):
        self.goff, self.keys, self.rank, self.box = goff, keys, rank, box
        self.sorted_lo, self.max_groups = sorted_lo, int(max_groups)


def kd_supported(cells: Cells) -> bool:
    if cells.keys is None or cells.S == 0:
        return False
    return _native.load().evr_cells_kd_limits(cells.stride, cells.m, cells.max_cells, None) == 0


def cells_kd_order(cells: Cells) -> KdGroups:
    if cells.keys is None:
        raise ValueError("cells_kd_order needs compressed cells (device box decomposition)")
    S, m, stride = cells.S, cells.m, cells.stride
    dev = cells.off.device
    ng = (cells.counts + 15) // 16
    goff_h = np.zeros(S + 1, dtype=np.int64)
    np.cumsum(ng, out=goff_h[1:])
    G = int(goff_h[-1])
    goff = torch.as_tensor(goff_h.astype(np.int32)).to(dev)
    keys = torch.empty(max(G, 1) * 16, dtype=torch.int64, device=dev)
    rank = torch.empty(max(G, 1) * m * 16, dtype=torch.int16, device=dev)
    box = torch.empty(max(G, 1) * 8, dtype=torch.int16, device=dev)
    sorted_lo = torch.empty(S, m, stride, dtype=torch.float64, device=dev)
    call("evr_cells_kd_order_device", _stream(), S, m, stride, cells.off.data_ptr(), goff.data_ptr(),
         cells.max_cells, cells.keys.data_ptr(), cells.pts.data_ptr(), cells.rank0.data_ptr(), keys.data_ptr(),
         rank.data_ptr(), box.data_ptr(), sorted_lo.data_ptr())
    cells.kd = KdGroups(goff, keys, rank, box, sorted_lo, int(ng.max()) if S else 0)
    return cells.kd


class BoxCapacityError(RuntimeError):
    """The device box decomposition needs more LUB slots than its capacity / memory bound
    (the caller falls back to the exact host partition)."""


def box_decompose_device(O: torch.Tensor, ref: torch.Tensor, cap: int = 16384, max_cap: int = 1 << 20,
                         max_workspace_bytes: int = 8 << 30) -> Cells:
    O, ref = _dev(O, "O"), _dev(ref, "ref")
    m, n, S = O.shape
    dev = O.device
    while True:
        nbytes = _native.load().evr_box_device_workspace_bytes(S, n, m, cap)
        if nbytes > max_workspace_bytes:
            raise BoxCapacityError(f"box decomposition: {cap} LUB slots x {S} samples need {nbytes} B of workspace")
        ws = torch.empty(nbytes, dtype=torch.uint8, device=dev)
        cs = torch.empty(2, S, dtype=torch.int32, device=dev)
        call("evr_box_decompose_device", _stream(), S, n, m, O.data_ptr(), ref.data_ptr(), cap, ws.data_ptr(),
             cs[0].data_ptr(), cs[1].data_ptr())
        h = cs.cpu().numpy()
        if not h[1].any():
            break
        if cap >= max_cap:
            raise BoxCapacityError(f"box decomposition: more than {max_cap} local upper bounds in one sample")
        cap *= 4
    counts = h[0].astype(np.int64)
    off_h = np.zeros(S + 1, dtype=np.int64)
    np.cumsum(counts, out=off_h[1:])
    total = int(off_h[-1])
    off = torch.as_tensor(off_h.astype(np.int32)).to(dev)
    stride = n + m
    keys = torch.empty(max(total, 1), dtype=torch.int64, device=dev)
    pts = torch.empty(S, stride, m, dtype=torch.float64, device=dev)
    rank0 = torch.empty(S, stride, dtype=torch.int32, device=dev)
    call("evr_box_pack_keys_device", _stream(), S, n, m, cap, ws.data_ptr(), off.data_ptr(),
         int(counts.max()) if S else 0, keys.data_ptr(), pts.data_ptr(), rank0.data_ptr())
    return Cells(off, counts, m, keys=keys, pts=pts, rank0=rank0, stride=stride)


def box_decompose_kd_device(O: torch.Tensor, ref: torch.Tensor, want_kd: bool = True, cap: int = 16384,
                            max_cap: int = 1 << 20, max_workspace_bytes: int = 8 << 30):
    O, ref = _dev(O, "O"), _dev(ref, "ref")
    m, n, S = O.shape
    dev = O.device
    stride = n + m
    lib = _native.load()
    counts_h = np.zeros(S, dtype=np.int32)
    info = np.zeros(3, dtype=np.int32)
    cap0 = cap
    while True:
        nbytes = lib.evr_box_device_workspace_bytes(S, n, m, cap)
        G = S * cap // 16 + S
        out_bytes = 8 * S * cap + 8 * S * stride * m + 4 * S * stride + 16 * S + 8
        if want_kd:
            out_bytes += G * 16 * 8 + G * m * 16 * 2 + G * 8 * 2 + 8 * S * m * stride
        if nbytes + out_bytes > max_workspace_bytes:
            raise BoxCapacityError(f"box decomposition: {cap} LUB slots x {S} samples need {nbytes + out_bytes} B "
                                   "of workspace and outputs")
        try:
            ws = torch.empty(nbytes, dtype=torch.uint8, device=dev)
            cs = torch.empty(2, S, dtype=torch.int32, device=dev)
            offs = torch.empty(2, S + 1, dtype=torch.int32, device=dev)
            keys = torch.empty(S * cap, dtype=torch.int64, device=dev)
            pts = torch.empty(S, stride, m, dtype=torch.float64, device=dev)
            rank0 = torch.empty(S, stride, dtype=torch.int32, device=dev)
            if want_kd:
                okeys = torch.empty(G * 16, dtype=torch.int64, device=dev)
                ork = torch.empty(G * m * 16, dtype=torch.int16, device=dev)
                ogb = torch.empty(G * 8, dtype=torch.int16, device=dev)
                osv = torch.empty(S, m, stride, dtype=torch.float64, device=dev)
            else:
                okeys = ork = ogb = osv = None
        except torch.OutOfMemoryError as e:
            raise BoxCapacityError(f"box decomposition: out of device memory at {cap} LUB slots x {S} samples") from e
        call("evr_box_kd_pipeline", _stream(), S, n, m, O.data_ptr(), ref.data_ptr(), cap, ws.data_ptr(),
             cs[0].data_ptr(), cs[1].data_ptr(), offs[0].data_ptr(), offs[1].data_ptr(), keys.data_ptr(),
             pts.data_ptr(), rank0.data_ptr(), int(bool(want_kd)), _p(okeys), _p(ork), _p(ogb), _p(osv),
             counts_h.ctypes.data, info.ctypes.data)
        if not info[0]:
            break
        if cap >= max_cap:
            raise BoxCapacityError(f"box decomposition: more than {max_cap} local upper bounds in one sample")
        cap *= 4
    counts = counts_h.astype(np.int64)
    total = int(counts.sum())
    del ws
    trim = (lambda t: t.clone()) if cap > cap0 else (lambda t: t)
    cells = Cells(offs[0], counts, m, keys=trim(keys[:max(total, 1)]), pts=pts, rank0=rank0, stride=stride)
    if info[1]:
        ng = (counts + 15) // 16
        Gu = int(ng.sum())
        cells.kd = KdGroups(offs[1], trim(okeys[:max(Gu, 1) * 16]), trim(ork[:max(Gu, 1) * m * 16]),
                            trim(ogb[:max(Gu, 1) * 8]), osv, int(ng.max()) if S else 0)
    return cells, bool(info[1])


_SOBOL_DIRECTIONS = {}


def _sobol_directions(dim: int) -> torch.Tensor:
    V = _SOBOL_DIRECTIONS.get(dim)
    if V is None:
        V = torch.zeros(dim, 30, dtype=torch.long)
        torch._sobol_engine_initialize_state_(V, dim)
        if len(_SOBOL_DIRECTIONS) > 16:
            _SOBOL_DIRECTIONS.clear()
        _SOBOL_DIRECTIONS[dim] = V
    return V


SOBOL_MAXDIM = 21201


def _iid_normal(n: int, dim: int, seed: int, device, d0: int, nd: int, layout: int, m: int) -> torch.Tensor:
    warnings.warn(f"{dim} base-sample dims exceed SobolEngine.MAXDIM={SOBOL_MAXDIM}: IID normal base samples",
                  RuntimeWarning)
    g = torch.Generator().manual_seed(int(seed))
    Z = torch.randn(n, dim, generator=g, dtype=torch.float64)[:, d0:d0 + nd]
    if layout == 0:
        return Z.contiguous().to(device)
    return Z.reshape(n, nd // m, m).permute(2, 1, 0).contiguous().to(device)


def sobol_scramble(dim: int, seed: int, d0: int = 0, nd: Optional[int] = None):
    nd = dim - d0 if nd is None else nd
    if not (0 <= d0 and nd >= 1 and d0 + nd <= dim):
        raise ValueError("sobol_scramble: dims out of range")
    if dim > SOBOL_MAXDIM:
        return None
    V, shift = _pinned_scramble_out(dim, d0, nd)
    call("evr_sobol_scramble_range", dim, int(seed), d0, nd, V.data_ptr(), shift.data_ptr())
    return V, shift


def _pinned_scramble_out(dim: int, d0: int, nd: int):
    pin = os.environ.get("EVR_SOBOL_PINNED", "1") != "0" and torch.cuda.is_available()
    V = torch.empty(nd, 30, dtype=torch.long, pin_memory=pin)
    V.copy_(_sobol_directions(dim)[d0:d0 + nd])
    return V, torch.empty(nd, dtype=torch.long, pin_memory=pin)


class SobolStream:

    def __init__(self, seed: int, max_dim: int):
        lib = _native.load()
        self._lib = lib
        self.seed, self.max_dim = int(seed), int(max_dim)
        h = ctypes.c_void_p()
        call("evr_sobol_stream_create", self.seed, lib.evr_sobol_stream_words(self.max_dim), ctypes.byref(h))
        self._h = h

    def scramble(self, dim: int, d0: int = 0, nd: Optional[int] = None):
        nd = dim - d0 if nd is None else nd
        if dim > SOBOL_MAXDIM or dim > self.max_dim or nd < 1:
            return None
        V, shift = _pinned_scramble_out(dim, d0, nd)
        call("evr_sobol_scramble_stream", self._h, dim, d0, nd, V.data_ptr(), shift.data_ptr())
        return V, shift

    def __del__(self):
        h = getattr(self, "_h", None)
        if h is not None:
            try:
                self._lib.evr_sobol_stream_destroy(h)
            except Exception:
                pass
            self._h = None


def sobol_normal(n: int, dim: int, seed: int, device, d0: int = 0, nd: Optional[int] = None,
                 layout: int = 0, m: int = 1, scrambled=None) -> torch.Tensor:
    nd = dim - d0 if nd is None else nd
    if not (0 <= d0 and d0 + nd <= dim):
        raise ValueError("sobol_normal: dims out of range")
    if dim > SOBOL_MAXDIM:
        return _iid_normal(n, dim, seed, device, d0, nd, layout, m)
    if layout == 0:
        out = torch.empty(n, nd, dtype=torch.float64, device=device)
    else:
        out = torch.empty(m, nd // m, n, dtype=torch.float64, device=device)
    if nd == 0:
        return out
    V, shift = scrambled if scrambled is not None else sobol_scramble(dim, seed, d0, nd)
    Vd = V.to(device, non_blocking=V.is_pinned())
    sd = shift.to(device, non_blocking=shift.is_pinned())
    call("evr_sobol_normal", _stream(), n, nd, 0, Vd.data_ptr(), sd.data_ptr(), layout, m, out.data_ptr())
    return out


def box_decompose(obj: np.ndarray, ref: np.ndarray, mask: Optional[np.ndarray] = None, num_threads: int = 0,
                  layout: str = "jis", alpha: float = 0.0):
    lib = _native.load()
    obj = np.ascontiguousarray(obj, dtype=np.float64)
    if layout == "jis":
        m, n, S = obj.shape
        ss, si, sj = 1, S, n * S
    elif layout == "sij":
        S, n, m = obj.shape
        ss, si, sj = n * m, m, 1
    else:
        raise ValueError(layout)
    ref = np.ascontiguousarray(ref, dtype=np.float64)
    mk = None if mask is None else np.ascontiguousarray(mask, dtype=np.uint8)
    handle = ctypes.c_void_p()
    _native.check(lib.evr_box_decompose_approx(S, n, m, obj.ctypes.data, ss, si, sj,
                                               None if mk is None else mk.ctypes.data, ref.ctypes.data,
                                               float(alpha), int(num_threads), ctypes.byref(handle)),
                  "evr_box_decompose_approx")
    try:
        total = lib.evr_cells_total(handle)
        lo = np.empty((total, m), dtype=np.float64)
        hi = np.empty((total, m), dtype=np.float64)
        off = np.empty(S + 1, dtype=np.int32)
        lib.evr_cells_copy(handle, lo.ctypes.data, hi.ctypes.data, off.ctypes.data)
    finally:
        lib.evr_cells_free(handle)
    return lo, hi, off


def device_arch(device: int = 0) -> str:
    buf = ctypes.create_string_buffer(64)
    call("evr_device_arch", device, buf, 64)
    return buf.value.decode()
```

### include/everest_amd.h

```cpp
#ifndef EVEREST_AMD_H
#define EVEREST_AMD_H

#ifdef __cplusplus
extern "C" {
#endif

#define EVR_VERSION 1

#define EVR_KERNEL_RBF 0
#define EVR_KERNEL_MATERN05 1
#define EVR_KERNEL_MATERN15 2
#define EVR_KERNEL_MATERN25 3
#define EVR_KERNEL_MIXED 16

int evr_version(void);
const char* evr_last_error(void);
int evr_device_arch(int device, char* buf, int buflen);
int evr_stream_sync(void* stream);

int evr_kernel_matrix(void* stream, int kind, int B, int n1, int n2, int d,
                      const double* X1, const double* shift1, const double* scale1,
                      const double* X2, const double* shift2, const double* scale2,
                      const double* lengthscales, const double* outputscale,
                      const double* diag_add, double* K);

int evr_kernel_cross_grad(void* stream, int kind, int B, int n1, int n2, int d,
                          const double* X1, const double* shift1, const double* scale1,
                          const double* X2, const double* shift2, const double* scale2,
                          const double* lengthscales, const double* outputscale,
                          const double* G, double* dX2, double* work);
long long evr_kernel_cross_grad_workspace_doubles(int n1, int n2, int d);

int evr_kernel_lengthscale_grad(void* stream, int kind, int B, int n, int d, const double* X,
                                const double* lengthscales, const double* W, double* gls,
                                double* work);
int evr_gp_mll_terms(void* stream, int B, int n, const double* L, const double* Linv,
                     const double* r, const double* alpha, double* out);

typedef struct evr_mll_plan evr_mll_plan;
int evr_mll_plan_create(void* stream, int kind, int B, int n, int d, const double* Xn, const double* Y,
                        evr_mll_plan** out);
int evr_mll_plan_eval(void* stream, evr_mll_plan* plan, const double* params, double* out);
void evr_mll_plan_destroy(evr_mll_plan* plan);

int evr_mll_fit_rounds(void* stream, evr_mll_plan* plan, void** runs, int* task, double* x, double* f, double* g,
                       int* nit, int* nfev, int* status, int maxiter, int maxfun, const double* prior, double* params,
                       int* pending);
int evr_mll_assemble(int B, int n, int d, const double* prior, const double* x, const double* terms,
                     const double* gls, double* ll, double* g);
int evr_lbfgsb_advance(void* run, double f, const double* g, double* x, int* task, int* nit, int* nfev,
                       int* status, int maxiter, int maxfun);

int evr_gemm_f64(void* stream, int transA, int transB, int M, int N, int K, double alpha,
                 const double* A, int lda, long long strideA, const double* B, int ldb,
                 long long strideB, double beta, double* C, int ldc, long long strideC, int batch);

int evr_cholesky(void* stream, int batch, int n, const double* A, int lda, long long strideA,
                 double* L, int ldl, long long strideL, double jitter0, int max_tries,
                 double* jitter_used, int* info);

int evr_cholesky_inverse(void* stream, int batch, int n, const double* A, int lda, long long strideA,
                         double* L, int ldl, long long strideL, double* Linv, int ldi,
                         long long strideI, double jitter0, int max_tries, double* jitter_used,
                         int* info);

int evr_trsm_lower(void* stream, int batch, int n, int nrhs, const double* L, int ldl,
                   long long strideL, int transpose, double* B, int ldb, long long strideB);
int evr_tri_inv_lower(void* stream, int batch, int n, const double* L, int ldl, long long strideL,
                      double* Linv, int ldi, long long strideI);

int evr_gp_posterior_finalize(void* stream, int B, int n, int nt, const double* R,
                              const double* c, const double* ym, const double* ys,
                              const double* kxx, const double* noise_add,
                              double* mean, double* var);

long long evr_gp_posterior_workspace_doubles(int B, int n, int nt);
int evr_gp_posterior(void* stream, int B, int n, int nt, int d, int kind, const double* Xn, const double* X,
                     const double* shift, const double* scale, const double* lengthscales, const double* M,
                     const double* c, const double* ym, const double* ys, const double* kxx,
                     const double* noise_add, double* mean, double* var, double* work);

typedef struct {
  int n, nb, S, m;
  const double* c;
  const double* ym;
  const double* ys;
  const double* kxx;
  const double* zq;
  const double* obj_a;
  const double* obj_b;
  const double* cell_lo;
  const double* cell_hi;
  const int* cell_off;
  int max_cells;
  const unsigned long long* cell_keys;
  const double* cell_pts;
  const int* cell_rank0;
  int pts_stride;
  const int* grp_off;
  const unsigned long long* grp_keys;
  const unsigned short* grp_rank;
  const unsigned short* grp_box;
  const double* sorted_lo;
  int max_groups;
  unsigned long long* scan_counters;
  int no_h;
  int log_hvi;
  double tau_relu, tau_max;
} evr_qnehvi_state;

int evr_qnehvi_samples(void* stream, const evr_qnehvi_state* st, int b, const double* R,
                       double* G, double* L22, int* flags);
long long evr_hvi_workspace_doubles(const evr_qnehvi_state* st, int b, int backward);
int evr_hvi_forward(void* stream, const evr_qnehvi_state* st, int b, const double* G,
                    const int* flags, double* work, double* acq);
int evr_mean_over_samples(void* stream, int S, int b, const double* partial, double* acq);
int evr_hvi_backward(void* stream, const evr_qnehvi_state* st, int b, const double* G,
                     const double* gout, double* work, double* dG);
int evr_hvi_forward_backward(void* stream, const evr_qnehvi_state* st, int b, const double* G,
                             const int* flags, const double* gout, double* work, double* acq,
                             double* dG);
int evr_hvi_restart_fb_applies(const evr_qnehvi_state* st, int b);
int evr_hvi_scan_limits(int stride, int m);
int evr_hvi_restart_fb(void* stream, const evr_qnehvi_state* st, int b, const double* G, double* sval,
                       double* dG);
int evr_qnehvi_samples_backward(void* stream, const evr_qnehvi_state* st, int b, const double* R,
                                const double* L22, const double* dG, double* gR);

int evr_qnehvi_norms_rows(const evr_qnehvi_state* st);
int evr_qnehvi_project(void* stream, const evr_qnehvi_state* st, int b, const double* M, const double* Kx,
                       double* R, double* norms, double* work);
long long evr_qnehvi_project_workspace_doubles(const evr_qnehvi_state* st, int b);
int evr_qnehvi_samples_norms(void* stream, const evr_qnehvi_state* st, int b, const double* R,
                             const double* norms, double* G, double* L22, int* flags);
int evr_qnehvi_project_backward(void* stream, const evr_qnehvi_state* st, int b, const double* M,
                                const double* R, const double* L22, const double* dG, double* dKx,
                                double* work);
long long evr_qnehvi_project_backward_workspace_doubles(const evr_qnehvi_state* st, int b);

typedef struct {
  int n, d, kind;
  const double* Xn;
  const double* lengthscales;
  const double* shift;
  const double* scale;
  const double* M;
} evr_qnehvi_model;
typedef struct evr_qnehvi_plan evr_qnehvi_plan;
long long evr_qnehvi_plan_workspace_bytes(const evr_qnehvi_state* st, const evr_qnehvi_model* md, int b,
                                          int backward);
int evr_qnehvi_plan_create(void* stream, const evr_qnehvi_state* st, const evr_qnehvi_model* md, int b,
                           int backward, const double* X, void* work, double* acq, double* dX, int use_graph,
                           evr_qnehvi_plan** out);
int evr_qnehvi_small_applies(const evr_qnehvi_state* st, int b, int d);
long long evr_qnehvi_small_workspace_doubles(const evr_qnehvi_state* st, int b, int d, int which);
int evr_qnehvi_small_forward(void* stream, const evr_qnehvi_state* st, const evr_qnehvi_model* md, int b,
                             const double* Kx, double* R, double* P);
int evr_qnehvi_small_samples(void* stream, const evr_qnehvi_state* st, int b, const double* R, const double* P,
                             double* G, double* L22, int* flags);
int evr_qnehvi_small_backward(void* stream, const evr_qnehvi_state* st, const evr_qnehvi_model* md, int b,
                              const double* X, const double* R, const double* L22, const double* dG, double* dXp,
                              double* dX);
int evr_qnehvi_plan_run(void* stream, evr_qnehvi_plan* plan);
int evr_qnehvi_plan_eval_host(void* stream, evr_qnehvi_plan* plan, const double* x, double* out);
void evr_qnehvi_plan_destroy(evr_qnehvi_plan* plan);

#define EVR_LBFGSB_FG 1
#define EVR_LBFGSB_NEW_X 2
#define EVR_LBFGSB_CONV_PGTOL 3
#define EVR_LBFGSB_CONV_FACTR 4
#define EVR_LBFGSB_ABNORMAL 5
#define EVR_LBFGSB_ERROR 6
typedef struct evr_lbfgsb evr_lbfgsb;
int evr_lbfgsb_create(int n, int m, const double* lb, const double* ub, double factr, double pgtol, int maxls,
                      evr_lbfgsb** out);
int evr_lbfgsb_start(evr_lbfgsb* h, const double* x0, double* x);
int evr_lbfgsb_step(evr_lbfgsb* h, double f, const double* g, double* x);
void evr_lbfgsb_stats(const evr_lbfgsb* h, int* nit, int* nfev, double* f, double* pgnorm);
void evr_lbfgsb_destroy(evr_lbfgsb* h);

int evr_hit_and_run(int d, int rows, const double* A, const double* b, int k, const double* N,
                    const double* x0, long long n, unsigned long long seed, long long n_burnin,
                    long long n_thinning, double* out);

#define EVR_ERR_NOTPSD 7
int evr_qnehvi_plan_minimize(void* stream, evr_qnehvi_plan* plan, const double* x0, const double* lb,
                             const double* ub, int maxiter, int maxfun, double factr, double pgtol, int m,
                             int maxls, double* x, double* acq, int* info);

#define EVR_OBJ_AFFINE 0
#define EVR_OBJ_CLOSE_TO_TARGET 1
#define EVR_QNG_MAX_Q 12
typedef struct {
  int q;
  int m_obj;
  const int* obj_out;
  const int* obj_kind;
  const double* obj_p0;
  const double* obj_p1;
  int n_con;
  const int* con_out;
  const double* con_sign;
  const double* con_thr;
  const double* con_eta;
  const double* zq;
} evr_qn_general;
long long evr_qng_workspace_doubles(const evr_qnehvi_state* stm, const evr_qnehvi_state* sth,
                                    const evr_qn_general* g, const evr_qnehvi_model* md, int b, int backward);
int evr_qng_eval(void* stream, const evr_qnehvi_state* stm, const evr_qnehvi_state* sth, const evr_qn_general* g,
                 const evr_qnehvi_model* md, int b, const double* X, const double* gout, double* work,
                 double* acq, double* dX);
long long evr_qlog_workspace_doubles(const evr_qnehvi_state* stm, const evr_qnehvi_state* sth, const evr_qn_general* g,
                                     const evr_qnehvi_model* md, int b, int backward);
int evr_qlog_eval(void* stream, const evr_qnehvi_state* stm, const evr_qnehvi_state* sth, const evr_qn_general* g,
                  const evr_qnehvi_model* md, int b, const double* X, const double* gout, double* work,
                  double* acq, double* dX);
int evr_objective_general(void* stream, int m_model, int n, int S, const evr_qn_general* g, const double* Y,
                          const double* mu, const double* ref, double* O);
int evr_objective_weights(void* stream, int m_model, int n, const evr_qn_general* g, const double* Y, double* G,
                          double* W);

int evr_nei_scan(void* stream, int q, int log, int S, int b, const double* Y, const double* best,
                 int best_stride, double obj_a, double obj_b, double tau_relu, double tau_max,
                 const int* flags, const double* gout, double* acq, double* dY);
typedef struct {
  int log;
  double tau_relu;
  double tau_max;
  const double* best;
  int best_stride;
} evr_nei;
long long evr_qnei_workspace_doubles(const evr_qnehvi_state* stm, const evr_qn_general* g,
                                     const evr_qnehvi_model* md, int b, int backward);
int evr_qnei_eval(void* stream, const evr_qnehvi_state* stm, const evr_qn_general* g, const evr_qnehvi_model* md,
                  const evr_nei* nei, int b, const double* X, const double* gout, double* work, double* acq,
                  double* dX);

#define EVR_OBJ_SIGMOID 2
#define EVR_OBJ_TARGET 3
#define EVR_SOBO_MAX_TERMS 8
typedef struct {
  int log;
  double tau_relu;
  double tau_max;
  const double* best;
  int best_stride;
  int n_term;
  const int* term_out;
  const int* term_kind;
  const double* term_w;
  const double* term_p0;
  const double* term_p1;
  const double* term_p2;
  int n_con;
  const int* con_out;
  const double* con_sign;
  const double* con_thr;
  const double* con_eta;
} evr_sobo;
int evr_sobo_scan(void* stream, int q, int m_model, int S, int b, const evr_sobo* sb, const double* Y,
                  const int* flags, const double* gout, double* acq, double* dY);
long long evr_qsobo_workspace_doubles(const evr_qnehvi_state* stm, const evr_qn_general* g,
                                      const evr_qnehvi_model* md, int b, int backward);
int evr_qsobo_eval(void* stream, const evr_qnehvi_state* stm, const evr_qn_general* g, const evr_qnehvi_model* md,
                   const evr_sobo* sb, int b, const double* X, const double* gout, double* work, double* acq,
                   double* dX);


int evr_qei(void* stream, int n, int b, int S, const double* R, double c, double ym, double ys,
            double kxx, const double* z, double obj_a, double obj_b, double best_f, double* acq,
            double* gR, int* flags);

int evr_pareto_mask(void* stream, int S, int n, int m, const double* O, const double* ref,
                    int dedup, unsigned char* mask, int* counts);

int evr_objective_affine(void* stream, int m, int n, int S, const double* Y, const double* mu,
                         const double* a, const double* b, double* O);
int evr_scale_batched(void* stream, int B, long long per, const double* alpha, double* X);
int evr_add_selection(void* stream, int B, int nb, int n, const int* idx, const double* val, double* E);

typedef struct evr_cells evr_cells;
int evr_box_decompose(int S, int n, int m, const double* obj, long long ss, long long si,
                      long long sj, const unsigned char* mask, const double* ref, int num_threads,
                      evr_cells** out);
int evr_box_decompose_approx(int S, int n, int m, const double* obj, long long ss, long long si,
                             long long sj, const unsigned char* mask, const double* ref, double alpha,
                             int num_threads, evr_cells** out);
long long evr_cells_total(const evr_cells* c);
int evr_cells_copy(const evr_cells* c, double* lo, double* hi, int* off);
void evr_cells_free(evr_cells* c);

int evr_box_device_limits(int n, int m, int* max_points, long long* lds_bytes);
long long evr_box_device_workspace_bytes(int S, int n, int m, int cap);
int evr_box_decompose_device(void* stream, int S, int n, int m, const double* obj, const double* ref,
                             int cap, void* work, int* counts, int* status);
int evr_box_pack_keys_device(void* stream, int S, int n, int m, int cap, const void* work,
                             const int* off, int max_cells, unsigned long long* keys, double* pts,
                             int* rank0);
int evr_cells_from_keys(void* stream, int S, int m, int stride, const int* off, int max_cells,
                        const unsigned long long* keys, const double* pts, const int* rank0,
                        double* lo, double* hi);

int evr_box_kd_pipeline(void* stream, int S, int n, int m, const double* obj, const double* ref, int cap,
                        void* work, int* counts_dev, int* status_dev, int* off_dev, int* goff_dev,
                        unsigned long long* keys, double* pts, int* rank0, int want_kd, unsigned long long* okeys,
                        unsigned short* ork, unsigned short* ogb, double* osv, int* counts_host, int* info);
int evr_cells_kd_limits(int stride, int m, int max_cells, long long* lds_bytes);
int evr_cells_kd_order_device(void* stream, int S, int m, int stride, const int* off, const int* goff,
                              int max_cells, const unsigned long long* keys, const double* pts,
                              const int* rank0, unsigned long long* okeys, unsigned short* ork,
                              unsigned short* ogb, double* osv);

int evr_sobol_scramble(int dim, unsigned long long seed, long long* V, long long* shift);
int evr_sobol_scramble_range(int dim, unsigned long long seed, int d0, int nd, long long* V, long long* shift);
typedef struct evr_sobol_stream evr_sobol_stream;
long long evr_sobol_stream_words(int dim);
int evr_sobol_stream_create(unsigned long long seed, long long nwords, evr_sobol_stream** out);
int evr_sobol_scramble_stream(const evr_sobol_stream* st, int dim, int d0, int nd, long long* V, long long* shift);
void evr_sobol_stream_destroy(evr_sobol_stream* st);
int evr_sobol_normal(void* stream, int n, int nd, int d0, const long long* V, const long long* shift,
                     int layout, int m, double* out);

#ifdef __cplusplus
}
#endif
#endif
```

Before: 202,100 candidates/s.

## Move qNEHVI construction into a single native driver with overlapped operator build

Adds a native evr_qnehvi_construct entry point that runs baseline pruning, baseline posterior/Cholesky, Sobol sample generation, box decomposition and operator construction in one C++/HIP driver. A hook in the box-kd pipeline lets the operator build run on the stream while the box decomposition is in flight. This is meant to cut the many Python-side launches, syncs and host round-trips of the per-ask construction phase, which is part of ask() wall time. The cost is a large new native path that has to reproduce the Python construction exactly, with fallbacks for overflow and unsupported configurations.

```diff
diff --git a/everest_amd/_native.py b/everest_amd/_native.py
--- a/everest_amd/_native.py
+++ b/everest_amd/_native.py
@@ -60,6 +60,26 @@
         ("term_p1", c_void_p), ("term_p2", c_void_p),
         ("n_con", c_int),
         ("con_out", c_void_p), ("con_sign", c_void_p), ("con_thr", c_void_p), ("con_eta", c_void_p),
+    ]
+
+
+class EvrQnehviConstructArgs(ctypes.Structure):
+    _fields_ = [
+        ("stream", c_void_p), ("struct_bytes", c_int),
+        ("n", c_int), ("d", c_int), ("m", c_int), ("kind", c_int), ("nc", c_int), ("S", c_int),
+        ("prune_samples", c_int), ("max_points", c_int), ("cap", c_int), ("host_threads", c_int),
+        ("prune_seed", ctypes.c_ulonglong), ("sampler_seed", ctypes.c_ulonglong), ("prune_scrambled", c_int),
+        ("Xn", c_void_p), ("lengthscales", c_void_p), ("Linv", c_void_p), ("alpha", c_void_p), ("ym", c_void_p),
+        ("ys", c_void_p), ("c", c_void_p), ("obj_a", c_void_p), ("obj_b", c_void_p), ("ref", c_void_p),
+        ("Vdir", c_void_p), ("Vp", c_void_p), ("shift_p", c_void_p), ("Vb", c_void_p), ("shift_b", c_void_p),
+        ("Vq", c_void_p), ("shift_q", c_void_p), ("work", c_void_p),
+        ("M", c_void_p), ("zq", c_void_p), ("L_base", c_void_p), ("jitter", c_void_p), ("Zb", c_void_p),
+        ("Ob", c_void_p),
+        ("box_work", c_void_p), ("box_counts", c_void_p), ("box_status", c_void_p), ("cell_off", c_void_p),
+        ("grp_off", c_void_p), ("cell_keys", c_void_p), ("cell_pts", c_void_p), ("cell_rank0", c_void_p),
+        ("grp_keys", c_void_p), ("grp_rank", c_void_p), ("grp_box", c_void_p), ("sorted_lo", c_void_p),
+        ("nb", c_void_p), ("keep", c_void_p), ("prune_counts", c_void_p), ("cell_counts", c_void_p),
+        ("info", c_void_p), ("times", c_void_p),
     ]
 
 
@@ -184,6 +204,9 @@
     "evr_cells_kd_limits": ([c_int, c_int, c_int, c_void_p], c_int),
     "evr_cells_kd_order_device": ([c_void_p, c_int, c_int, c_int, c_void_p, c_void_p, c_int] + [c_void_p] * 7,
                                   c_int),
+    "evr_qnehvi_construct_workspace_bytes": ([c_int, c_int, c_int, c_int, c_int], c_longlong),
+    "evr_qnehvi_construct": ([POINTER(EvrQnehviConstructArgs)], c_int),
+    "evr_prune_select": ([c_int, c_void_p, c_int, c_void_p, c_void_p], c_int),
     "evr_sobol_scramble": ([c_int, ctypes.c_ulonglong, c_void_p, c_void_p], c_int),
     "evr_sobol_scramble_range": ([c_int, ctypes.c_ulonglong, c_int, c_int, c_void_p, c_void_p], c_int),
     "evr_sobol_stream_words": ([c_int], ctypes.c_longlong),
diff --git a/everest_amd/acquisition.py b/everest_amd/acquisition.py
--- a/everest_amd/acquisition.py
+++ b/everest_amd/acquisition.py
@@ -83,6 +83,18 @@
     return ops.Cells(torch.arange(S + 1, dtype=torch.int32, device=dev), np.ones(S, dtype=np.int64), m,
                      lo=ref.unsqueeze(0).repeat(S, 1).contiguous(),
                      hi=torch.full((S, m), math.inf, dtype=torch.float64, device=dev))
+
+
+def _kd_path(cells: ops.Cells, kd_built: bool, kd_scan) -> str:
+    if kd_built:
+        return "device+kd"
+    if kd_scan if kd_scan is not None else ops.kd_supported(cells):
+        ops.cells_kd_order(cells)
+        return "device+kd"
+    if kd_scan is None:
+        warnings.warn(f"{int(cells.counts.max())} cells in one sample exceed the sparse kd scan's limit; "
+                      "using the dense tiled scan (~10x slower)", RuntimeWarning)
+    return "device"
 
 
 def _decompose(O: torch.Tensor, ref: torch.Tensor, box_device=None, kd_scan=None, num_threads=None,
@@ -106,16 +118,7 @@
             warnings.warn(f"{e}; using the exact host partition", RuntimeWarning)
             cells = None
         if cells is not None:
-            path = "device"
-            if kd_built:
-                path = "device+kd"
-            elif kd_scan if kd_scan is not None else ops.kd_supported(cells):
-                ops.cells_kd_order(cells)
-                path = "device+kd"
-            elif kd_scan is None:
-                warnings.warn(f"{int(cells.counts.max())} cells in one sample exceed the sparse kd scan's limit; "
-                              "using the dense tiled scan (~10x slower)", RuntimeWarning)
-            return cells, path
+            return cells, _kd_path(cells, kd_built, kd_scan)
     elif not approx and box_device is None:
         warnings.warn(f"{P} points x {m} objectives exceed the device box decomposition's limits; "
                       "using the host partition", RuntimeWarning)
@@ -240,6 +243,19 @@
     @property
     def supports_plan(self) -> bool:
         return self.spec.affine_identity and self._pending_rows() is None
+
+    @staticmethod
+    def native_construct_applies(gp, spec: ops.GeneralSpec, nc: int, leading: bool, npend: int, root: str,
+                                 prune_baseline: bool, explicit_samples: bool, box_device, kd_scan,
+                                 alpha: float) -> bool:
+        m = gp.B
+        return bool(npend == 0 and root == "split" and spec.affine_identity and prune_baseline and leading
+                    and nc >= 1 and not explicit_samples and alpha == 0.0 and box_device in (None, True)
+                    and kd_scan in (None, True) and getattr(gp, "mask", None) is None
+                    and os.environ.get("EVR_BOX_PIPELINE", "1") != "0"
+                    and os.environ.get("EVR_CONSTRUCTION_PROBES") != "1"
+                    and (nc + 1) * m <= ops.SOBOL_MAXDIM
+                    and ops.box_device_supported(nc, m) and ops.hvi_scan_supported(nc + m, m))
 
     def _init_general(self, spec: ops.GeneralSpec, cells, nk: int, nb_rows: int, no_h: bool = False):
         gp, m = self.gp, self.m
@@ -476,7 +492,9 @@
                 and np.array_equal(X_baseline_raw, X_train_raw[:nbl]) and _distinct_rows(X_baseline_raw)
                 and all_rows[:nbl].all()):
             base_rows = np.arange(nbl, dtype=np.int64)
+            leading = True
         else:
+            leading = False
             first = {}
             for i, row in enumerate(map(tuple, X_train_raw)):
                 if all_rows[i]:
@@ -496,9 +514,19 @@
         nk = n + npend
         self.nk = nk
 
+        root = root or os.environ.get("EVR_ROOT", "split")
+        if root not in ("fused", "split"):
+            raise ValueError(f"root must be 'fused' or 'split', got {root!r}")
+
         import time as _time
         tm = {}
         t0 = _time.perf_counter()
+        if self.native_construct_applies(gp, spec, nbl, leading, npend, root, prune_baseline,
+                                         not (z_prune is None and z_base_full is None and z_new_full is None),
+                                         box_device, kd_scan, alpha):
+            self._construct_native(nbl, prune_seed, prune_samples, max_frac, box_device, kd_scan, num_threads, alpha,
+                                   tm, t0)
+            return
         _probe_on = os.environ.get("EVR_CONSTRUCTION_PROBES") == "1"
         _last = [t0]
 
@@ -600,9 +628,6 @@
             join_box = lambda: (cells0, "none")
         probe("box")
 
-        root = root or os.environ.get("EVR_ROOT", "split")
-        if root not in ("fused", "split"):
-            raise ValueError(f"root must be 'fused' or 'split', got {root!r}")
         fused = root == "fused" and nb > 0
         self.root = "fused" if fused else "split"
         nb_rows = 0 if fused else nb
@@ -644,11 +669,21 @@
         cells, self.box_path = join_box()
         if nb > 0:
             tm["box_decomposition"] = _time.perf_counter() - t1
+        self._finish_construct(cells, M, Rr, nb_rows, probs)
+        probe("operator")
+        self._plans = {}
+        torch.cuda.synchronize(dev)
+        tm["total"] = _time.perf_counter() - t0
+        self.timings = tm
+
+    def _finish_construct(self, cells, M: torch.Tensor, Rr: int, nb_rows: int, probs, copy_alpha: bool = True):
+        gp, spec, m, n, nk, nb, S_ = self.gp, self.spec, self.m, self.n, self.nk, self.nb, self.S
         self.cells = cells
         counts_c = cells.counts
         self.stats = ConstructionStats(n_train=n, n_base=nb, total_cells=int(np.sum(counts_c)),
                                        max_cells=int(counts_c.max()) if len(counts_c) else 0, prune_probs=probs)
-        M[:, Rr - 1, :n].copy_(gp.alpha)
+        if copy_alpha:
+            M[:, Rr - 1, :n].copy_(gp.alpha)
         self.M = M
         self.state = ops.make_state(nk, nb_rows, S_, m, gp.const, gp.ym, gp.ys, gp.kxx, self.zq, self.obj_a,
                                     self.obj_b, cells)
@@ -661,12 +696,38 @@
         self.model = _native.EvrQnehviModel(n=nk, d=gp.d, kind=gp.kind, Xn=self.Xk.data_ptr(), lengthscales=gp.ls.data_ptr(),
                                             shift=self._lo_c.data_ptr(), scale=self._scale_c.data_ptr(),
                                             M=self.M.data_ptr())
-        probe("operator")
+
+    def _construct_native(self, nc: int, prune_seed: int, prune_samples: int, max_frac: float, box_device, kd_scan,
+                          num_threads, alpha: float, tm: dict, t0: float):
+        import time as _time
+        gp, m, n, S_ = self.gp, self.m, self.n, self.S
+        fut = _PREFETCHED.pop((nc * m, int(prune_seed), 0, nc * m), None)
+        t_in = _time.perf_counter() - t0
+        r = ops.qnehvi_construct(gp.Xn, gp.ls, gp.kind, gp.Linv, gp.alpha, gp.ym, gp.ys, gp.const, self.obj_a,
+                                 self.obj_b, self.ref, nc, S_, prune_samples, math.ceil(max_frac * nc), prune_seed,
+                                 self.sampler_seed, prune_scrambled=_result(fut), host_threads=_host_threads())
+        probs = r.prune_counts.astype(np.float64) / prune_samples
+        nb = r.nb
+        self.nb, self.base_rows = nb, r.keep
+        self.zq, self.root = r.zq, "split"
+        tm["prune"] = t_in + float(r.times[0])
+        if nb > 0:
+            self.L_base, self.base_jitter, self._Zb = r.L_base, r.jitter, r.Zb
+            tm["baseline"] = float(r.times[1])
+            tm["box_decomposition"] = float(r.times[2])
+            if r.overflow:
+                cells, self.box_path = _decompose(r.Ob, self.ref, box_device, kd_scan, num_threads, alpha)
+            else:
+                cells, self.box_path = r.cells, _kd_path(r.cells, r.kd_built, kd_scan)
+        else:
+            cells, self.box_path = _single_cell(self.ref, S_, self.spec.m_obj), "none"
+        Rr = n + nb + S_ + 1
+        self.Rr = Rr
+        self._finish_construct(cells, r.M, Rr, nb, probs, copy_alpha=False)
         self._plans = {}
-        torch.cuda.synchronize(dev)
+        torch.cuda.synchronize(self.dev)
         tm["total"] = _time.perf_counter() - t0
         self.timings = tm
-
 
     def z_base_host(self) -> Optional[torch.Tensor]:
         zb = getattr(self, "_Zb", None)
diff --git a/everest_amd/csrc/box_device.hip b/everest_amd/csrc/box_device.hip
--- a/everest_amd/csrc/box_device.hip
+++ b/everest_amd/csrc/box_device.hip
@@ -442,6 +442,18 @@
                         void* work, int* counts_dev, int* status_dev, int* off_dev, int* goff_dev,
                         unsigned long long* keys, double* pts, int* rank0, int want_kd, unsigned long long* okeys,
                         unsigned short* ork, unsigned short* ogb, double* osv, int* counts_host, int* info) {
+  return evr::box_kd_pipeline_hooked(stream, S, n, m, obj, ref, cap, work, counts_dev, status_dev, off_dev, goff_dev,
+                                     keys, pts, rank0, want_kd, okeys, ork, ogb, osv, counts_host, info, nullptr,
+                                     nullptr);
+}
+
+}
+
+int evr::box_kd_pipeline_hooked(void* stream, int S, int n, int m, const double* obj, const double* ref, int cap,
+                                void* work, int* counts_dev, int* status_dev, int* off_dev, int* goff_dev,
+                                unsigned long long* keys, double* pts, int* rank0, int want_kd,
+                                unsigned long long* okeys, unsigned short* ork, unsigned short* ogb, double* osv,
+                                int* counts_host, int* info, int (*after_build)(void*), void* hook_arg) {
   EVR_CHECK(S >= 1 && counts_dev && status_dev && off_dev && goff_dev && keys && pts && rank0 && counts_host &&
                 info && (!want_kd || (okeys && ork && ogb && osv)),
             "evr_box_kd_pipeline: bad arguments");
@@ -475,6 +487,8 @@
   int* hoff = stage + 2 * S;
   int* hgoff = hoff + S + 1;
   if (int rc = box_decompose_launch(stream, S, n, m, obj, ref, cap, work, counts_dev, status_dev, stage_d)) return rc;
+  if (after_build)
+    if (int rc = after_build(hook_arg)) return rc;
   EVR_HIP(hipStreamSynchronize(s));
   info[0] = info[1] = info[2] = 0;
   int maxc = 0;
@@ -510,5 +524,3 @@
   EVR_HIP(hipEventRecord(copied, s));
   return 0;
 }
-
-}
diff --git a/everest_amd/csrc/common.hpp b/everest_amd/csrc/common.hpp
--- a/everest_amd/csrc/common.hpp
+++ b/everest_amd/csrc/common.hpp
@@ -41,6 +41,12 @@
   } while (0)
 
 inline int cdiv(long long a, long long b) { return (int)((a + b - 1) / b); }
+
+int box_kd_pipeline_hooked(void* stream, int S, int n, int m, const double* obj, const double* ref, int cap,
+                           void* work, int* counts_dev, int* status_dev, int* off_dev, int* goff_dev,
+                           unsigned long long* keys, double* pts, int* rank0, int want_kd,
+                           unsigned long long* okeys, unsigned short* ork, unsigned short* ogb, double* osv,
+                           int* counts_host, int* info, int (*after_build)(void*), void* hook_arg);
 
 __device__ __forceinline__ int xcd_swizzle(int orig, int nwg) {
   const int xcd = orig & 7, q = nwg >> 3, r = nwg & 7;
diff --git a/everest_amd/csrc/qnehvi_construct.hip b/everest_amd/csrc/qnehvi_construct.hip
--- /dev/null
+++ b/everest_amd/csrc/qnehvi_construct.hip
@@ -0,0 +1,473 @@
+#include <algorithm>
+#include <chrono>
+#include <condition_variable>
+#include <deque>
+#include <functional>
+#include <future>
+#include <memory>
+#include <mutex>
+#include <numeric>
+#include <thread>
+#include <vector>
+
+#include "../../include/everest_amd.h"
+#include "common.hpp"
+
+namespace {
+using namespace evr;
+
+__global__ void qc_mu_train_kernel(int m, int n, const double* __restrict__ mu_t, const double* __restrict__ ym,
+                                   const double* __restrict__ ys, const double* __restrict__ c,
+                                   double* __restrict__ mu_train, double* __restrict__ ys2) {
+#pragma clang fp contract(off)
+  const long long e = (long long)blockIdx.x * 256 + threadIdx.x;
+  if (e < (long long)m * n) {
+    const int b = (int)(e / n);
+    const double t = c[b] + mu_t[e];
+    const double u = ys[b] * t;
+    mu_train[e] = ym[b] + u;
+  }
+  if (e < m) ys2[e] = ys[e] * ys[e];
+}
+
+__global__ void qc_gather_sym_kernel(int n, int k, const int* __restrict__ rows, const double* __restrict__ in,
+                                     double* __restrict__ out) {
+  const long long e = (long long)blockIdx.x * 256 + threadIdx.x;
+  if (e >= (long long)k * k) return;
+  const int i = (int)(e / k), j = (int)(e % k), b = blockIdx.y;
+  out[(size_t)b * k * k + e] = in[((size_t)b * n + rows[i]) * n + rows[j]];
+}
+
+__global__ void qc_gather_cols_kernel(int nr, int n, int k, const int* __restrict__ rows,
+                                      const double* __restrict__ in, double* __restrict__ out) {
+  const long long e = (long long)blockIdx.x * 256 + threadIdx.x;
+  if (e >= (long long)nr * k) return;
+  const int r = (int)(e / k), j = (int)(e % k), b = blockIdx.y;
+  out[(size_t)b * nr * k + e] = in[((size_t)b * nr + r) * n + rows[j]];
+}
+
+__global__ void qc_copy_block_kernel(long long per, const double* __restrict__ src, long long src_stride,
+                                     double* __restrict__ dst, long long dst_stride) {
+  const long long e = (long long)blockIdx.x * 256 + threadIdx.x;
+  if (e >= per) return;
+  dst[(size_t)blockIdx.y * dst_stride + e] = src[(size_t)blockIdx.y * src_stride + e];
+}
+
+__global__ void qc_zero_block_kernel(long long per, double* __restrict__ dst, long long dst_stride) {
+  const long long e = (long long)blockIdx.x * 256 + threadIdx.x;
+  if (e >= per) return;
+  dst[(size_t)blockIdx.y * dst_stride + e] = 0.0;
+}
+
+__global__ void qc_zero_int_kernel(int n, int* __restrict__ dst) {
+  const int e = blockIdx.x * 256 + threadIdx.x;
+  if (e < n) dst[e] = 0;
+}
+
+inline size_t al(size_t bytes) { return (bytes + 255) & ~(size_t)255; }
+
+struct QcLayout {
+  size_t K, A, mu_t, mu_train, ys2, Sig_c, mu_c, Lp, Zp, Yp, Op, Sig_b, mu_b, Yb, A_b, E, jit_p;
+  size_t info_p, info_b, counts, idx, iota;
+  size_t Vd_p, sd_p, Vd_b, sd_b, Vd_q, sd_q;
+  size_t bytes;
+};
+
+QcLayout qc_layout(int n, int m, int nc, int S, int Sp) {
+  QcLayout L;
+  size_t o = 0;
+  auto take = [&](size_t bytes) {
+    const size_t at = o;
+    o += al(bytes);
+    return at;
+  };
+  const size_t D = sizeof(double), I = sizeof(int), Q = sizeof(long long);
+  const size_t mn = (size_t)m * n, mnn = mn * n, mcc = (size_t)m * nc * nc, mc = (size_t)m * nc;
+  L.K = take(D * mnn);
+  L.A = take(D * mnn);
+  L.mu_t = take(D * mn);
+  L.mu_train = take(D * mn);
+  L.ys2 = take(D * m);
+  L.Sig_c = take(D * mcc);
+  L.mu_c = take(D * mc);
+  L.Lp = take(D * mcc);
+  L.Zp = take(D * mc * Sp);
+  L.Yp = take(D * mc * Sp);
+  L.Op = take(D * mc * Sp);
+  L.Sig_b = take(D * mcc);
+  L.mu_b = take(D * mc);
+  L.Yb = take(D * mc * S);
+  L.A_b = take(D * mn * nc);
+  L.E = take(D * mc * n);
+  L.jit_p = take(D * m);
+  L.info_p = take(I * m);
+  L.info_b = take(I * m);
+  L.counts = take(I * nc);
+  L.idx = take(I * nc);
+  L.iota = take(I * nc);
+  L.Vd_p = take(Q * mc * 30);
+  L.sd_p = take(Q * mc);
+  L.Vd_b = take(Q * mc * 30);
+  L.sd_b = take(Q * mc);
+  L.Vd_q = take(Q * (size_t)m * 30);
+  L.sd_q = take(Q * m);
+  L.bytes = o;
+  return L;
+}
+
+struct QcHost {
+  int dev = -1;
+  hipStream_t side = nullptr;
+  hipEvent_t entry = nullptr, draw_p = nullptr, draw_b = nullptr, ob = nullptr, box = nullptr;
+  int* stage = nullptr;
+  size_t stage_n = 0;
+};
+
+int qc_host(QcHost** out, size_t need) {
+  thread_local QcHost H;
+  int dev = 0;
+  EVR_HIP(hipGetDevice(&dev));
+  if (H.dev != dev) {
+    H = QcHost();
+    EVR_HIP(hipStreamCreateWithFlags(&H.side, hipStreamNonBlocking));
+    for (hipEvent_t* e : {&H.entry, &H.draw_p, &H.draw_b, &H.ob, &H.box})
+      EVR_HIP(hipEventCreateWithFlags(e, hipEventDisableTiming));
+    H.dev = dev;
+  }
+  if (H.stage_n < need) {
+    if (H.stage) (void)hipHostFree(H.stage);
+    H.stage = nullptr;
+    H.stage_n = 0;
+    EVR_HIP(hipHostMalloc((void**)&H.stage, sizeof(int) * need, hipHostMallocDefault));
+    H.stage_n = need;
+  }
+  *out = &H;
+  return 0;
+}
+
+class Worker {
+ public:
+  Worker() { std::thread([this] { loop(); }).detach(); }
+  std::future<int> submit(std::function<int()> f) {
+    auto task = std::make_shared<std::packaged_task<int()>>(std::move(f));
+    std::future<int> fut = task->get_future();
+    {
+      std::lock_guard<std::mutex> lk(mu_);
+      q_.push_back([task] { (*task)(); });
+    }
+    cv_.notify_one();
+    return fut;
+  }
+
+ private:
+  void loop() {
+    for (;;) {
+      std::function<void()> job;
+      {
+        std::unique_lock<std::mutex> lk(mu_);
+        cv_.wait(lk, [&] { return !q_.empty(); });
+        job = std::move(q_.front());
+        q_.pop_front();
+      }
+      job();
+    }
+  }
+  std::mutex mu_;
+  std::condition_variable cv_;
+  std::deque<std::function<void()>> q_;
+};
+Worker& worker(int i) {
+  static Worker* W = new Worker[3];
+  return W[i];
+}
+
+struct Pending {
+  std::vector<std::future<int>*> f;
+  ~Pending() {
+    for (std::future<int>* x : f)
+      if (x->valid()) x->wait();
+  }
+};
+
+double now_s() {
+  return std::chrono::duration<double>(std::chrono::steady_clock::now().time_since_epoch()).count();
+}
+
+struct QcOperator {
+  const evr_qnehvi_construct_args* a;
+  const QcLayout* L;
+  unsigned char* w;
+  int nb;
+  const int* rows;
+  bool identity;
+  const double* A_b;
+};
+
+int qc_operator(void* arg) {
+  const QcOperator& o = *(const QcOperator*)arg;
+  const evr_qnehvi_construct_args& a = *o.a;
+  hipStream_t s = (hipStream_t)a.stream;
+  const int n = a.n, m = a.m, S = a.S, nb = o.nb;
+  const long long Rr = (long long)n + nb + S + 1, sM = Rr * n;
+  double* E = (double*)(o.w + o.L->E);
+  const double* ys2 = (const double*)(o.w + o.L->ys2);
+  if (int rc = evr_gemm_f64(s, 1, 0, nb, n, n, -1.0, o.A_b, o.identity ? n : nb, (long long)n * (o.identity ? n : nb),
+                            a.Linv, n, (long long)n * n, 0.0, E, n, (long long)nb * n, m))
+    return rc;
+  if (int rc = evr_add_selection(s, m, nb, n, o.rows, nullptr, E)) return rc;
+  if (int rc = evr_scale_batched(s, m, (long long)nb * n, ys2, E)) return rc;
+  if (int rc = evr_trsm_lower(s, m, nb, n, a.L_base, nb, (long long)nb * nb, 0, E, n, (long long)nb * n)) return rc;
+  if (int rc = evr_gemm_f64(s, 1, 0, S, n, nb, 1.0, a.Zb, S, (long long)nb * S, E, n, (long long)nb * n, 0.0,
+                            a.M + (size_t)(n + nb) * n, n, sM, m))
+    return rc;
+  qc_copy_block_kernel<<<dim3(cdiv((long long)nb * n, 256), m), 256, 0, s>>>((long long)nb * n, E, (long long)nb * n,
+                                                                            a.M + (size_t)n * n, sM);
+  EVR_LAUNCH_CHECK();
+  return 0;
+}
+
+}
+
+using namespace evr;
+
+extern "C" {
+
+int evr_prune_select(int nc, const int* counts, int max_points, long long* keep, int* nb) {
+  EVR_CHECK(nc >= 0 && counts && keep && nb && max_points >= 0, "evr_prune_select: bad arguments");
+  std::vector<int> k;
+  for (int i = 0; i < nc; ++i)
+    if (counts[i] != 0) k.push_back(i);
+  if ((int)k.size() > max_points) {
+    std::vector<int> order(nc);
+    std::iota(order.begin(), order.end(), 0);
+    std::stable_sort(order.begin(), order.end(), [&](int x, int y) { return counts[x] > counts[y]; });
+    k.assign(order.begin(), order.begin() + max_points);
+    std::sort(k.begin(), k.end());
+  }
+  for (size_t i = 0; i < k.size(); ++i) keep[i] = k[i];
+  *nb = (int)k.size();
+  return 0;
+}
+
+long long evr_qnehvi_construct_workspace_bytes(int n, int m, int nc, int S, int prune_samples) {
+  if (n < 1 || m < 1 || nc < 1 || nc > n || S < 1 || prune_samples < 1) return 0;
+  return (long long)qc_layout(n, m, nc, S, prune_samples).bytes;
+}
+
+int evr_qnehvi_construct(const evr_qnehvi_construct_args* ap) {
+  EVR_CHECK(ap, "evr_qnehvi_construct: bad arguments");
+  const evr_qnehvi_construct_args& a = *ap;
+  EVR_CHECK(a.struct_bytes == (int)sizeof(evr_qnehvi_construct_args),
+            "evr_qnehvi_construct: argument struct of %d bytes, this library expects %d", a.struct_bytes,
+            (int)sizeof(evr_qnehvi_construct_args));
+  const int n = a.n, m = a.m, nc = a.nc, S = a.S, Sp = a.prune_samples;
+  EVR_CHECK(n >= 1 && a.d >= 1 && m >= 1 && m <= 8 && nc >= 1 && nc <= n && S >= 1 && Sp >= 1 && a.max_points >= 0 &&
+                a.Xn && a.lengthscales && a.Linv && a.alpha && a.ym && a.ys && a.c && a.obj_a && a.obj_b && a.ref &&
+                a.Vdir && a.Vp && a.shift_p && a.Vb && a.shift_b && a.Vq && a.shift_q && a.work && a.M && a.zq &&
+                a.L_base && a.jitter && a.Zb && a.Ob && a.box_work && a.box_counts && a.box_status && a.cell_off &&
+                a.grp_off && a.cell_keys && a.cell_pts && a.cell_rank0 && a.grp_keys && a.grp_rank && a.grp_box &&
+                a.sorted_lo && a.keep && a.prune_counts && a.cell_counts && a.info && a.times && a.nb,
+            "evr_qnehvi_construct: bad arguments");
+  EVR_CHECK((long long)(nc + 1) * m <= 21201, "evr_qnehvi_construct: %d base-sample dims exceed the Sobol engine's",
+            (nc + 1) * m);
+  EVR_CHECK(evr_box_device_limits(nc, m, nullptr, nullptr) == 0 && evr_hvi_scan_limits(nc + m, m) == 0,
+            "evr_qnehvi_construct: %d points x %d objectives exceed the device box decomposition's limits", nc, m);
+  const double t0 = now_s();
+  hipStream_t s = (hipStream_t)a.stream;
+  const QcLayout L = qc_layout(n, m, nc, S, Sp);
+  unsigned char* w = (unsigned char*)a.work;
+  auto dp = [&](size_t off) { return (double*)(w + off); };
+  auto ip = [&](size_t off) { return (int*)(w + off); };
+  auto qp = [&](size_t off) { return (long long*)(w + off); };
+  QcHost* H = nullptr;
+  if (int rc = qc_host(&H, (size_t)3 * nc + 2 * m)) return rc;
+  int* h_idx = H->stage;
+  int* h_iota = h_idx + nc;
+  int* h_counts = h_iota + nc;
+  int* h_info = h_counts + nc;
+  const int dev = H->dev;
+  hipStream_t side = H->side;
+  a.info[0] = a.info[1] = a.info[2] = 0;
+  *a.nb = 0;
+
+  EVR_HIP(hipEventRecord(H->entry, s));
+  EVR_HIP(hipStreamWaitEvent(side, H->entry, 0));
+
+  const int dim_p = nc * m, max_dim = (nc + 1) * m;
+  std::promise<void> p_scrambled;
+  std::shared_future<void> f_scrambled = p_scrambled.get_future().share();
+  evr_sobol_stream* sob = nullptr;
+  struct StreamGuard {
+    evr_sobol_stream** st;
+    ~StreamGuard() {
+      if (*st) evr_sobol_stream_destroy(*st);
+    }
+  } stream_guard{&sob};
+  std::future<int> f_draw_p, f_stream, f_draw_b, f_scr_b;
+  Pending pending{{&f_draw_p, &f_stream, &f_draw_b, &f_scr_b}};
+  f_draw_p = worker(0).submit([&]() -> int {
+    bool told = false;
+    auto body = [&]() -> int {
+      EVR_HIP(hipSetDevice(dev));
+      if (!a.prune_scrambled) {
+        std::memcpy(a.Vp, a.Vdir, sizeof(long long) * (size_t)dim_p * 30);
+        if (int rc = evr_sobol_scramble_range(dim_p, a.prune_seed, 0, dim_p, a.Vp, a.shift_p)) return rc;
+      }
+      p_scrambled.set_value();
+      told = true;
+      EVR_HIP(hipMemcpyAsync(qp(L.Vd_p), a.Vp, sizeof(long long) * (size_t)dim_p * 30, hipMemcpyHostToDevice, side));
+      EVR_HIP(hipMemcpyAsync(qp(L.sd_p), a.shift_p, sizeof(long long) * dim_p, hipMemcpyHostToDevice, side));
+      if (int rc = evr_sobol_normal(side, Sp, dim_p, 0, qp(L.Vd_p), qp(L.sd_p), 1, m, dp(L.Zp))) return rc;
+      EVR_HIP(hipEventRecord(H->draw_p, side));
+      return 0;
+    };
+    const int rc = body();
+    if (!told) p_scrambled.set_value();
+    return rc;
+  });
+  const bool serial_host = a.host_threads < 4;
+  f_stream = worker(1).submit([&, serial_host]() -> int {
+    if (serial_host) f_scrambled.wait();
+    return evr_sobol_stream_create(a.sampler_seed, evr_sobol_stream_words(max_dim), &sob);
+  });
+
+  double *K = dp(L.K), *A = dp(L.A), *mu_train = dp(L.mu_train), *ys2 = dp(L.ys2);
+  const long long nn = (long long)n * n;
+  if (int rc = evr_kernel_matrix(s, a.kind, m, n, n, a.d, a.Xn, nullptr, nullptr, a.Xn, nullptr, nullptr,
+                                 a.lengthscales, nullptr, nullptr, K))
+    return rc;
+  if (int rc = evr_gemm_f64(s, 0, 0, n, 1, n, 1.0, K, n, nn, a.alpha, 1, n, 0.0, dp(L.mu_t), 1, n, m)) return rc;
+  qc_mu_train_kernel<<<cdiv((long long)m * n, 256), 256, 0, s>>>(m, n, dp(L.mu_t), a.ym, a.ys, a.c, mu_train, ys2);
+  EVR_LAUNCH_CHECK();
+  if (int rc = evr_gemm_f64(s, 0, 0, n, n, n, 1.0, a.Linv, n, nn, K, n, nn, 0.0, A, n, nn, m)) return rc;
+  if (int rc = evr_gemm_f64(s, 1, 0, n, n, n, -1.0, A, n, nn, A, n, nn, 1.0, K, n, nn, m)) return rc;
+  if (int rc = evr_scale_batched(s, m, nn, ys2, K)) return rc;
+  const double* Sig = K;
+
+  for (int i = 0; i < nc; ++i) h_iota[i] = i;
+  const double *Sig_c = Sig, *mu_c = mu_train;
+  if (nc < n) {
+    EVR_HIP(hipMemcpyAsync(ip(L.iota), h_iota, sizeof(int) * nc, hipMemcpyHostToDevice, s));
+    qc_gather_sym_kernel<<<dim3(cdiv((long long)nc * nc, 256), m), 256, 0, s>>>(n, nc, ip(L.iota), Sig, dp(L.Sig_c));
+    EVR_LAUNCH_CHECK();
+    qc_gather_cols_kernel<<<dim3(cdiv(nc, 256), m), 256, 0, s>>>(1, n, nc, ip(L.iota), mu_train, dp(L.mu_c));
+    EVR_LAUNCH_CHECK();
+    Sig_c = dp(L.Sig_c);
+    mu_c = dp(L.mu_c);
+  }
+  const long long cc = (long long)nc * nc;
+  if (int rc = evr_cholesky(s, m, nc, Sig_c, nc, cc, dp(L.Lp), nc, cc, 1e-8, 3, dp(L.jit_p), ip(L.info_p))) return rc;
+  if (int rc = f_draw_p.get()) return rc;
+  EVR_HIP(hipStreamWaitEvent(s, H->draw_p, 0));
+  if (int rc = evr_gemm_f64(s, 0, 0, nc, Sp, nc, 1.0, dp(L.Lp), nc, cc, dp(L.Zp), Sp, (long long)nc * Sp, 0.0,
+                            dp(L.Yp), Sp, (long long)nc * Sp, m))
+    return rc;
+  if (int rc = evr_objective_affine(s, m, nc, Sp, dp(L.Yp), mu_c, a.obj_a, a.obj_b, dp(L.Op))) return rc;
+  qc_zero_int_kernel<<<cdiv(nc, 256), 256, 0, s>>>(nc, ip(L.counts));
+  EVR_LAUNCH_CHECK();
+  if (int rc = evr_pareto_mask(s, Sp, nc, m, dp(L.Op), a.ref, 0, nullptr, ip(L.counts))) return rc;
+  EVR_HIP(hipMemcpyAsync(h_counts, ip(L.counts), sizeof(int) * nc, hipMemcpyDeviceToHost, s));
+  EVR_HIP(hipMemcpyAsync(h_info, ip(L.info_p), sizeof(int) * m, hipMemcpyDeviceToHost, s));
+  EVR_HIP(hipStreamSynchronize(s));
+  for (int b = 0; b < m; ++b)
+    if (h_info[b]) {
+      set_error("evr_qnehvi_construct: prune covariance of output %d not positive definite after the jitter ladder", b);
+      return EVR_ERR_NOTPSD;
+    }
+  std::memcpy(a.prune_counts, h_counts, sizeof(int) * nc);
+  int nb = 0;
+  if (int rc = evr_prune_select(nc, h_counts, a.max_points, a.keep, &nb)) return rc;
+  *a.nb = nb;
+  a.times[0] = now_s() - t0;
+  const bool identity = nb == n;
+  for (int i = 0; i < nb; ++i) h_idx[i] = (int)a.keep[i];
+
+  f_draw_b = worker(2).submit([&]() -> int {
+    EVR_HIP(hipSetDevice(dev));
+    if (int rc = f_stream.get()) return rc;
+    if (nb > 0)
+      f_scr_b = worker(0).submit([&]() -> int {
+        std::memcpy(a.Vb, a.Vdir, sizeof(long long) * (size_t)nb * m * 30);
+        return evr_sobol_scramble_stream(sob, nb * m, 0, nb * m, a.Vb, a.shift_b);
+      });
+    std::memcpy(a.Vq, a.Vdir + (size_t)nb * m * 30, sizeof(long long) * (size_t)m * 30);
+    if (int rc = evr_sobol_scramble_stream(sob, (nb + 1) * m, nb * m, m, a.Vq, a.shift_q)) return rc;
+    EVR_HIP(hipMemcpyAsync(qp(L.Vd_q), a.Vq, sizeof(long long) * (size_t)m * 30, hipMemcpyHostToDevice, side));
+    EVR_HIP(hipMemcpyAsync(qp(L.sd_q), a.shift_q, sizeof(long long) * m, hipMemcpyHostToDevice, side));
+    if (int rc = evr_sobol_normal(side, S, m, 0, qp(L.Vd_q), qp(L.sd_q), 0, 1, a.zq)) return rc;
+    if (nb > 0) {
+      if (int rc = f_scr_b.get()) return rc;
+      EVR_HIP(hipMemcpyAsync(qp(L.Vd_b), a.Vb, sizeof(long long) * (size_t)nb * m * 30, hipMemcpyHostToDevice, side));
+      EVR_HIP(hipMemcpyAsync(qp(L.sd_b), a.shift_b, sizeof(long long) * nb * m, hipMemcpyHostToDevice, side));
+      if (int rc = evr_sobol_normal(side, S, nb * m, 0, qp(L.Vd_b), qp(L.sd_b), 1, m, a.Zb)) return rc;
+    }
+    EVR_HIP(hipEventRecord(H->draw_b, side));
+    return 0;
+  });
+
+  const long long Rr = (long long)n + nb + S + 1, sM = Rr * n;
+  qc_copy_block_kernel<<<dim3(cdiv(nn, 256), m), 256, 0, s>>>(nn, a.Linv, nn, a.M, sM);
+  EVR_LAUNCH_CHECK();
+  qc_copy_block_kernel<<<dim3(cdiv(n, 256), m), 256, 0, s>>>(n, a.alpha, n, a.M + (size_t)(Rr - 1) * n, sM);
+  EVR_LAUNCH_CHECK();
+
+  if (nb == 0) {
+    qc_zero_block_kernel<<<dim3(cdiv((long long)S * n, 256), m), 256, 0, s>>>((long long)S * n, a.M + (size_t)n * n,
+                                                                              sM);
+    EVR_LAUNCH_CHECK();
+    if (int rc = f_draw_b.get()) return rc;
+    EVR_HIP(hipStreamWaitEvent(s, H->draw_b, 0));
+    EVR_HIP(hipStreamSynchronize(s));
+    a.times[1] = a.times[2] = 0.0;
+    a.times[3] = now_s() - t0;
+    return 0;
+  }
+
+  const int* rows = ip(L.idx);
+  EVR_HIP(hipMemcpyAsync(ip(L.idx), h_idx, sizeof(int) * nb, hipMemcpyHostToDevice, s));
+  const double *Sig_b = Sig, *mu_b = mu_train, *A_b = A;
+  if (!identity) {
+    qc_gather_sym_kernel<<<dim3(cdiv((long long)nb * nb, 256), m), 256, 0, s>>>(n, nb, rows, Sig, dp(L.Sig_b));
+    EVR_LAUNCH_CHECK();
+    qc_gather_cols_kernel<<<dim3(cdiv(nb, 256), m), 256, 0, s>>>(1, n, nb, rows, mu_train, dp(L.mu_b));
+    EVR_LAUNCH_CHECK();
+    qc_gather_cols_kernel<<<dim3(cdiv((long long)n * nb, 256), m), 256, 0, s>>>(n, n, nb, rows, A, dp(L.A_b));
+    EVR_LAUNCH_CHECK();
+    Sig_b = dp(L.Sig_b);
+    mu_b = dp(L.mu_b);
+    A_b = dp(L.A_b);
+  }
+  const long long bb = (long long)nb * nb;
+  if (int rc = evr_cholesky(s, m, nb, Sig_b, nb, bb, a.L_base, nb, bb, 1e-8, 3, a.jitter, ip(L.info_b))) return rc;
+  if (int rc = f_draw_b.get()) return rc;
+  EVR_HIP(hipStreamWaitEvent(s, H->draw_b, 0));
+  if (int rc = evr_gemm_f64(s, 0, 0, nb, S, nb, 1.0, a.L_base, nb, bb, a.Zb, S, (long long)nb * S, 0.0, dp(L.Yb), S,
+                            (long long)nb * S, m))
+    return rc;
+  if (int rc = evr_objective_affine(s, m, nb, S, dp(L.Yb), mu_b, a.obj_a, a.obj_b, a.Ob)) return rc;
+  EVR_HIP(hipEventRecord(H->ob, s));
+  a.times[1] = now_s() - t0 - a.times[0];
+  const double t1 = now_s();
+
+  EVR_HIP(hipStreamWaitEvent(side, H->ob, 0));
+  QcOperator op{&a, &L, w, nb, rows, identity, A_b};
+  if (int rc = box_kd_pipeline_hooked(side, S, nb, m, a.Ob, a.ref, a.cap, a.box_work, a.box_counts, a.box_status,
+                                      a.cell_off, a.grp_off, a.cell_keys, a.cell_pts, a.cell_rank0, 1, a.grp_keys,
+                                      a.grp_rank, a.grp_box, a.sorted_lo, a.cell_counts, a.info, qc_operator, &op))
+    return rc;
+  EVR_HIP(hipEventRecord(H->box, side));
+  EVR_HIP(hipStreamWaitEvent(s, H->box, 0));
+  EVR_HIP(hipMemcpyAsync(h_info + m, ip(L.info_b), sizeof(int) * m, hipMemcpyDeviceToHost, s));
+  EVR_HIP(hipStreamSynchronize(s));
+  a.times[2] = now_s() - t1;
+  for (int b = 0; b < m; ++b)
+    if (h_info[m + b]) {
+      set_error("evr_qnehvi_construct: baseline covariance of output %d not positive definite after the jitter ladder",
+                b);
+      return EVR_ERR_NOTPSD;
+    }
+  a.times[3] = now_s() - t0;
+  return 0;
+}
+
+}
diff --git a/everest_amd/ops.py b/everest_amd/ops.py
--- a/everest_amd/ops.py
+++ b/everest_amd/ops.py
@@ -944,6 +944,116 @@
     return cells, bool(info[1])
 
 
+def prune_select(counts: np.ndarray, max_points: int) -> np.ndarray:
+    counts = np.ascontiguousarray(counts, dtype=np.int32)
+    keep = np.empty(max(counts.shape[0], 1), dtype=np.int64)
+    nb = ctypes.c_int(0)
+    call("evr_prune_select", counts.shape[0], counts.ctypes.data, int(max_points), keep.ctypes.data,
+         ctypes.addressof(nb))
+    return keep[:nb.value].copy()
+
+
+class QnehviConstruction:
+    """What evr_qnehvi_construct returns: the operator M, the new point's base samples zq, the
+    baseline root / jitter / base samples / objective samples, the kept rows and prune counts,
+    the cells (None without a baseline, or when a sample overflowed the capacity: ``overflow``)
+    and the driver's split times."""
+
+
+def qnehvi_construct(Xn, lengthscales, kind: int, Linv, alpha, ym, ys, const, obj_a, obj_b, ref, nc: int, S: int,
+                     prune_samples: int, max_points: int, prune_seed: int, sampler_seed: int, prune_scrambled=None,
+                     host_threads: int = 16, cap: int = 16384) -> QnehviConstruction:
+    args = [_dev(t, "construct") for t in (Xn, lengthscales, Linv, alpha, ym, ys, const, obj_a, obj_b, ref)]
+    Xn, lengthscales, Linv, alpha, ym, ys, const, obj_a, obj_b, ref = args
+    m, n, _ = Linv.shape
+    d = Xn.shape[1]
+    dev = Xn.device
+    lib = _native.load()
+    f64 = dict(dtype=torch.float64, device=dev)
+    i32 = dict(dtype=torch.int32, device=dev)
+    stride = nc + m
+    G = S * cap // 16 + S
+    work = torch.empty(lib.evr_qnehvi_construct_workspace_bytes(n, m, nc, S, prune_samples), dtype=torch.uint8, device=dev)
+    Mf = torch.empty(m * (n + nc + S + 1) * n, **f64)
+    zq = torch.empty(S, m, **f64)
+    Lb = torch.empty(m * nc * nc, **f64)
+    jit = torch.empty(m, **f64)
+    Zb = torch.empty(m * nc * S, **f64)
+    Ob = torch.empty(m * nc * S, **f64)
+    ws = torch.empty(lib.evr_box_device_workspace_bytes(S, nc, m, cap), dtype=torch.uint8, device=dev)
+    cs = torch.empty(2, S, **i32)
+    offs = torch.empty(2, S + 1, **i32)
+    keys = torch.empty(S * cap, dtype=torch.int64, device=dev)
+    pts = torch.empty(S * stride * m, **f64)
+    rank0 = torch.empty(S * stride, **i32)
+    okeys = torch.empty(G * 16, dtype=torch.int64, device=dev)
+    ork = torch.empty(G * m * 16, dtype=torch.int16, device=dev)
+    ogb = torch.empty(G * 8, dtype=torch.int16, device=dev)
+    osv = torch.empty(S * m * stride, **f64)
+    pin = torch.cuda.is_available()
+    Vdir = _sobol_directions((nc + 1) * m)
+    dp = nc * m
+    host = torch.empty(31 * (dp + m) + (0 if prune_scrambled is not None else 31 * dp), dtype=torch.long,
+                       pin_memory=pin)
+    Vb, shb = host[:30 * dp].view(dp, 30), host[30 * dp:31 * dp]
+    Vq, shq = host[31 * dp:31 * dp + 30 * m].view(m, 30), host[31 * dp + 30 * m:31 * (dp + m)]
+    if prune_scrambled is not None:
+        Vp, shp = prune_scrambled
+    else:
+        Vp, shp = host[31 * (dp + m):31 * (dp + m) + 30 * dp].view(dp, 30), host[31 * (dp + m) + 30 * dp:]
+    nb_h = ctypes.c_int(0)
+    keep = np.zeros(nc, dtype=np.int64)
+    pcounts = np.zeros(nc, dtype=np.int32)
+    ccounts = np.zeros(S, dtype=np.int32)
+    info = np.zeros(3, dtype=np.int32)
+    times = np.zeros(4, dtype=np.float64)
+    a = _native.EvrQnehviConstructArgs(
+        stream=_stream(), struct_bytes=ctypes.sizeof(_native.EvrQnehviConstructArgs), n=n, d=d, m=m, kind=int(kind), nc=int(nc), S=int(S), prune_samples=int(prune_samples),
+        max_points=int(max_points), cap=int(cap), host_threads=int(host_threads), prune_seed=int(prune_seed),
+        sampler_seed=int(sampler_seed), prune_scrambled=int(prune_scrambled is not None),
+        Xn=Xn.data_ptr(), lengthscales=lengthscales.data_ptr(), Linv=Linv.data_ptr(), alpha=alpha.data_ptr(),
+        ym=ym.data_ptr(), ys=ys.data_ptr(), c=const.data_ptr(), obj_a=obj_a.data_ptr(), obj_b=obj_b.data_ptr(),
+        ref=ref.data_ptr(), Vdir=Vdir.data_ptr(), Vp=Vp.data_ptr(), shift_p=shp.data_ptr(), Vb=Vb.data_ptr(),
+        shift_b=shb.data_ptr(), Vq=Vq.data_ptr(), shift_q=shq.data_ptr(), work=work.data_ptr(),
+        M=Mf.data_ptr(), zq=zq.data_ptr(), L_base=Lb.data_ptr(), jitter=jit.data_ptr(), Zb=Zb.data_ptr(),
+        Ob=Ob.data_ptr(), box_work=ws.data_ptr(), box_counts=cs[0].data_ptr(), box_status=cs[1].data_ptr(),
+        cell_off=offs[0].data_ptr(), grp_off=offs[1].data_ptr(), cell_keys=keys.data_ptr(), cell_pts=pts.data_ptr(),
+        cell_rank0=rank0.data_ptr(), grp_keys=okeys.data_ptr(), grp_rank=ork.data_ptr(), grp_box=ogb.data_ptr(),
+        sorted_lo=osv.data_ptr(), nb=ctypes.addressof(nb_h), keep=keep.ctypes.data,
+        prune_counts=pcounts.ctypes.data, cell_counts=ccounts.ctypes.data, info=info.ctypes.data,
+        times=times.ctypes.data)
+    status = lib.evr_qnehvi_construct(ctypes.byref(a))
+    if status == 7:
+        raise NotPSDError(lib.evr_last_error().decode(errors="replace"))
+    _native.check(status, "evr_qnehvi_construct")
+    nb = int(nb_h.value)
+    r = QnehviConstruction()
+    r.nb, r.keep, r.prune_counts, r.times = nb, keep[:nb].copy(), pcounts, times
+    r.M = Mf[:m * (n + nb + S + 1) * n].view(m, n + nb + S + 1, n)
+    r.zq = zq
+    r.cells, r.kd_built, r.overflow = None, False, False
+    r.L_base = r.jitter = r.Zb = r.Ob = None
+    if nb == 0:
+        return r
+    r.L_base, r.jitter = Lb[:m * nb * nb].view(m, nb, nb), jit
+    r.Zb, r.Ob = Zb[:m * nb * S].view(m, nb, S), Ob[:m * nb * S].view(m, nb, S)
+    if info[0]:
+        r.overflow = True
+        return r
+    counts = ccounts.astype(np.int64)
+    total = int(counts.sum())
+    st = nb + m
+    r.cells = Cells(offs[0], counts, m, keys=keys[:max(total, 1)], pts=pts[:S * st * m].view(S, st, m),
+                    rank0=rank0[:S * st].view(S, st), stride=st)
+    if info[1]:
+        ng = (counts + 15) // 16
+        Gu = int(ng.sum())
+        r.cells.kd = KdGroups(offs[1], okeys[:max(Gu, 1) * 16], ork[:max(Gu, 1) * m * 16], ogb[:max(Gu, 1) * 8],
+                              osv[:S * m * st].view(S, m, st), int(ng.max()) if S else 0)
+        r.kd_built = True
+    return r
+
+
 _SOBOL_DIRECTIONS = {}
 
 
diff --git a/include/everest_amd.h b/include/everest_amd.h
--- a/include/everest_amd.h
+++ b/include/everest_amd.h
@@ -165,6 +165,45 @@
 int evr_qnehvi_plan_eval_host(void* stream, evr_qnehvi_plan* plan, const double* x, double* out);
 void evr_qnehvi_plan_destroy(evr_qnehvi_plan* plan);
 
+typedef struct {
+  void* stream;
+  int struct_bytes;
+  int n, d, m, kind;
+  int nc;
+  int S, prune_samples;
+  int max_points;
+  int cap;
+  int host_threads;
+  unsigned long long prune_seed, sampler_seed;
+  int prune_scrambled;
+  const double *Xn, *lengthscales, *Linv, *alpha, *ym, *ys, *c, *obj_a, *obj_b, *ref;
+  const long long* Vdir;
+  long long *Vp, *shift_p;
+  long long *Vb, *shift_b;
+  long long *Vq, *shift_q;
+  void* work;
+  double *M, *zq, *L_base, *jitter, *Zb;
+  double* Ob;
+  void* box_work;
+  int *box_counts, *box_status;
+  int *cell_off, *grp_off;
+  unsigned long long* cell_keys;
+  double* cell_pts;
+  int* cell_rank0;
+  unsigned long long* grp_keys;
+  unsigned short *grp_rank, *grp_box;
+  double* sorted_lo;
+  int* nb;
+  long long* keep;
+  int* prune_counts;
+  int* cell_counts;
+  int* info;
+  double* times;
+} evr_qnehvi_construct_args;
+long long evr_qnehvi_construct_workspace_bytes(int n, int m, int nc, int S, int prune_samples);
+int evr_qnehvi_construct(const evr_qnehvi_construct_args* args);
+int evr_prune_select(int nc, const int* counts, int max_points, long long* keep, int* nb);
+
 #define EVR_LBFGSB_FG 1
 #define EVR_LBFGSB_NEW_X 2
 #define EVR_LBFGSB_CONV_PGTOL 3
```

After: 212,600 candidates/s (median of 6 runs). 1.05x the previous value.
